# christoskokas/gtsam-vSLAM

Measured on AMD Instinct MI355X. Metric: frames/sec (extract+match+localBA), 1500 feat stereo 752x480, higher is better.
Workload: dtype u8/i32 (extract, match) + f64 (pose LM, local BA)

## Files before the change

gtsam-vslam_amd/csrc/ba.hip:

```cpp
#include "common.hpp"
#include "comm.hpp"
#include "dmath.hpp"
#include "ba_pool.hpp"
#include "ba_packed.hpp"
#include <algorithm>
#include <cmath>
#include <numeric>
#include <vector>
#include <atomic>
#include <condition_variable>
#include <functional>
#include <memory>
#include <mutex>
#include <thread>

namespace vslam {

struct BaEdge {
    int a, b, fa, fb;
    DPose measured;
    double r[6], Ja[36], Jb[36];
    double Haa[36], Hab[36], Hbb[36], ga[6], gb[6];
};

struct BaDev {
    int NF, Lp, F, K, NE, n;
    const int* facKf; const int* facFi; const int* facLp; const int* facLm;
    const double* facZ; const double* facIs; const uint8_t* facRight;
    double* facJ;
    const int* lpStart; const int* lpSlotStart; const int* slotStart; const int* slotFi; const int* lpOrig;
    DPose* poseCur; DPose* poseTrial; const int* fidx;
    double* lmCur; double* lmTrial;
    BaEdge* edges;
    double* S; double* rhs; double* Spart; double* Sedge; double* dP; double* dL;
    double* sums; double* partial;
    int* flags;
    double fx, fy, cx, cy, b;
    double* ctl;
    int NB, specLin, cand;
    int adaptive, nAct;
    double lambda;
    DPose* poseBase; double* lmBase; size_t lmStride;
    double* facJBase; size_t facJStride; double* SedgeBase; BaEdge* edgesBase;
    double* facJ2; double* Sedge2; BaEdge* edges2;
    size_t sysStride, spartStride, partialStride, dLStride;
    int solveKind;
    double* Lg;
    double* ctlHost;
};
enum { BA_SOLVE_MFMA64 = 0, BA_SOLVE_WAVE = 1, BA_SOLVE_MFMA = 2, BA_SOLVE_LARGE = 3 };

enum { CTL_LAMBDA = 0, CTL_ERROR = 1, CTL_CUR = 2, CTL_INIT_ERR = 3, CTL_INTS = 8, CTL_DOUBLES = 16 };
enum { CI_STATE = 0, CI_SEL = 1, CI_ITER = 2, CI_INNER = 3, CI_MAXIT = 4, CI_FIRST = 5, CI_NACT = 6, CI_ROUNDS = 7 };
enum { BA_LINEARIZE = 0, BA_TRY = 1, BA_DONE = 2 };
enum { BA_MAX_NB = 4, SUMS_CAND = 16, FLAG_COUNT = 1, FLAG_FAIL = 4 };
__device__ __forceinline__ int ba_slot(int sel, int c, int NB) {
    const int s = sel + 1 + c;
    return s > NB ? s - (NB + 1) : s;
}
__device__ __forceinline__ bool ba_enter(BaDev& D, int state, int c = 0) {
    const int* ci = (const int*)(D.ctl + CTL_INTS);
    if (ci[CI_STATE] != state) return false;
    D.nAct = ci[CI_NACT];
    if (c >= D.nAct) return false;
    const int sel = ci[CI_SEL], ts = ba_slot(sel, c, D.NB);
    D.cand = c;
    D.poseCur = D.poseBase + (size_t)sel * D.K; D.poseTrial = D.poseBase + (size_t)ts * D.K;
    D.lmCur = D.lmBase + (size_t)sel * D.lmStride; D.lmTrial = D.lmBase + (size_t)ts * D.lmStride;
    if (D.specLin) {
        const size_t se = (size_t)D.n * D.n + D.n;
        D.facJ = D.facJBase + (size_t)sel * D.facJStride; D.facJ2 = D.facJBase + (size_t)ts * D.facJStride;
        D.Sedge = D.SedgeBase + (size_t)sel * se; D.Sedge2 = D.SedgeBase + (size_t)ts * se;
        D.edges = D.edgesBase + (size_t)sel * D.NE; D.edges2 = D.edgesBase + (size_t)ts * D.NE;
    }
    D.S += (size_t)c * D.sysStride; D.rhs += (size_t)c * D.sysStride; D.Spart += (size_t)c * D.spartStride;
    D.dP += (size_t)c * D.n; D.dL += (size_t)c * D.dLStride; D.partial += (size_t)c * D.partialStride;
    double lam = D.ctl[CTL_LAMBDA];
    for (int i = 0; i < c; i++) lam *= 10.0;
    D.lambda = lam;
    return true;
}

constexpr int BA_SCHUR_WAVES = 16;
constexpr int BA_LDS_MAX_F = 20;
constexpr int BA_LDS_BYTES = 160 * 1024, BA_STATIC_LDS_RESERVE = 1024, BA_DYN_LDS_MAX = BA_LDS_BYTES - BA_STATIC_LDS_RESERVE;

__device__ __forceinline__ void ba_eval_fac(const BaDev& D, const DPose& T, const double* p, bool right,
                                            const double* z, double is, double* r, double* Jp, double* Jl) {
    const double d[3] = {p[0] - T.t[0], p[1] - T.t[1], p[2] - T.t[2]};
    double q[3];
    mat3T_vec(T.R, d, q);
    if (Jp) { for (int c = 0; c < 12; c++) Jp[c] = 0; for (int c = 0; c < 6; c++) Jl[c] = 0; }
    if (is == 0.0) { r[0] = r[1] = 0.0; return; }
    if (q[2] <= 0) { r[0] = r[1] = 2.0 * D.fx * is; return; }
    const double x = q[0], y = q[1], zz = q[2], iz = 1.0 / zz;
    const double xx = right ? x - D.b : x;
    r[0] = (D.fx * xx * iz + D.cx - z[0]) * is;
    r[1] = (D.fy * y * iz + D.cy - z[1]) * is;
    if (!Jp) return;
    const double al[2][3] = {{D.fx * iz, 0, -D.fx * xx * iz * iz}, {0, D.fy * iz, -D.fy * y * iz * iz}};
    const double Sk[3][3] = {{0, -zz, y}, {zz, 0, -x}, {-y, x, 0}};
    for (int a = 0; a < 2; a++)
        for (int c = 0; c < 3; c++) {
            Jp[a * 6 + c] = (al[a][0] * Sk[0][c] + al[a][1] * Sk[1][c] + al[a][2] * Sk[2][c]) * is;
            Jp[a * 6 + 3 + c] = -al[a][c] * is;
            Jl[a * 3 + c] = (al[a][0] * T.R[3 * c] + al[a][1] * T.R[3 * c + 1] + al[a][2] * T.R[3 * c + 2]) * is;
        }
}

__device__ __forceinline__ void ba_eval_edge(const BaEdge& e, const DPose& Ta, const DPose& Tb, double* r,
                                             double* Ja, double* Jb) {
    const double w = 1.0 / 0.01;
    DPose Tai, h, Mi, d;
    pose_inverse(Ta, Tai);
    pose_compose(Tai, Tb, h);
    pose_inverse(e.measured, Mi);
    pose_compose(Mi, h, d);
    pose3_logmap(d, r);
    for (int i = 0; i < 6; i++) r[i] *= w;
    if (!Ja) return;
    double Hl[36], Ad[36];
    DPose hi;
    pose3_logmap_derivative(d, Hl);
    pose_inverse(h, hi);
    pose3_adjoint(hi, Ad);
    for (int i = 0; i < 6; i++)
        for (int j = 0; j < 6; j++) {
            double s = 0;
            for (int k = 0; k < 6; k++) s += Hl[i * 6 + k] * Ad[k * 6 + j];
            Ja[i * 6 + j] = -s * w;
            Jb[i * 6 + j] = Hl[i * 6 + j] * w;
        }
}

__device__ __forceinline__ double ba_edge_linearize(BaEdge& out, const BaEdge& E, const DPose& Ta, const DPose& Tb,
                                                    double* sW, double* Sacc, int n, int tid) {
    double* Hl = sW; double* Ad = Hl + 36; double* Ja = Ad + 36; double* Jb = Ja + 36; double* rr = Jb + 36;
    const double w = 1.0 / 0.01;
    const int fa = E.fa, fb = E.fb;
    const int lane = tid & 63, wave = tid >> 6;
    double v = 0;
    if (lane == 0 && wave < 3) {
        DPose Tai, h;
        pose_inverse(Ta, Tai);
        pose_compose(Tai, Tb, h);
        if (wave == 2) {
            DPose hi;
            pose_inverse(h, hi);
            pose3_adjoint(hi, Ad);
        } else {
            DPose Mi, d;
            pose_inverse(E.measured, Mi);
            pose_compose(Mi, h, d);
            if (wave == 0) {
                double r[6];
                pose3_logmap(d, r);
                for (int i = 0; i < 6; i++) { r[i] *= w; rr[i] = r[i]; out.r[i] = r[i]; v += r[i] * r[i]; }
            } else pose3_logmap_derivative(d, Hl);
        }
    }
    __syncthreads();
    if (wave != 0) return 0.0;
    asm volatile("s_waitcnt lgkmcnt(0)" ::: "memory");
    const int i = lane / 6, j = lane % 6;
    if (lane < 36) {
// ... 45 lines not shown
    __syncthreads();
    if (tid < NV) {
        double s = 0;
        for (int w = 0; w < NW; w++) s += red[w * NV + tid];
        out[tid] = s;
    }
    __syncthreads();
}

__device__ __forceinline__ void ba_ctl(const BaDev& D, int mode, double relTol, double absTol) {
    double* c = D.ctl;
    int* ci = (int*)(D.ctl + CTL_INTS);
    if (mode == 0) {
        if (ci[CI_STATE] != BA_LINEARIZE) return;
        if (ci[CI_FIRST]) {
            ci[CI_FIRST] = 0;
            c[CTL_ERROR] = D.sums[0];
            c[CTL_INIT_ERR] = D.sums[0];
            ci[CI_STATE] = (!(c[CTL_ERROR] <= 0.0) && ci[CI_ITER] < ci[CI_MAXIT]) ? BA_TRY : BA_DONE;
        } else ci[CI_STATE] = BA_TRY;
        c[CTL_CUR] = c[CTL_ERROR];
        return;
    }
    if (ci[CI_STATE] != BA_TRY) return;
    ci[CI_ROUNDS]++;
    const int nAct = ci[CI_NACT];
    for (int cand = 0; cand < nAct; cand++) {
        const double error = c[CTL_ERROR];
        double lambda = c[CTL_LAMBDA];
        bool stepOk = false, stop = false;
        double newErr = INFINITY;
        const double linChange = error - D.sums[SUMS_CAND + 2 * cand];
        if (!D.flags[FLAG_FAIL + cand] && linChange >= 0) {
            newErr = D.sums[SUMS_CAND + 2 * cand + 1];
            const double costChange = error - newErr;
            if (linChange > DBL_EPSILON * error) stepOk = (costChange / linChange) > 1e-3;
            if (fabs(costChange) < relTol * error) stop = true;
        }
        bool endInner = false;
        if (stepOk) {
            ci[CI_SEL] = ba_slot(ci[CI_SEL], cand, D.NB);
            c[CTL_ERROR] = newErr;
            lambda = lambda / 10.0;
            c[CTL_LAMBDA] = lambda > 0.0 ? lambda : 0.0;
            ci[CI_ITER]++; ci[CI_INNER]++;
            endInner = true;
        } else if (!stop) {
            lambda *= 10.0;
            c[CTL_LAMBDA] = lambda;
            ci[CI_INNER]++;
            if (lambda >= 1e5) endInner = true;
        } else endInner = true;
        if (!endInner) continue;
        const double currentError = c[CTL_CUR], newError = c[CTL_ERROR];
        bool converged;
        if (newError <= 0.0) converged = true;
        else {
            const double absDec = currentError - newError, relDec = absDec / currentError;
            converged = (relDec <= relTol) || (absDec <= absTol);
        }
        ci[CI_STATE] = (ci[CI_ITER] < ci[CI_MAXIT] && !converged && isfinite(currentError)) ? BA_LINEARIZE : BA_DONE;
        if (D.specLin && ci[CI_STATE] == BA_LINEARIZE) {
            c[CTL_CUR] = c[CTL_ERROR];
            ci[CI_STATE] = BA_TRY;
        }
        ci[CI_NACT] = D.adaptive ? 1 : D.NB;
        return;
    }
    ci[CI_NACT] = D.NB;
}

__global__ __launch_bounds__(256) void k_ba_ctl(const BaDev* __restrict__ tab, int mode, double relTol, double absTol) {
    BaDev D = *lane_entry(tab, blockIdx.z);
    __shared__ int sZero;
    if (threadIdx.x == 0) {
        ba_ctl(D, mode, relTol, absTol);
        sZero = mode == 1 && ((const int*)(D.ctl + CTL_INTS))[CI_STATE] == BA_LINEARIZE;
    }
    __syncthreads();
    if (sZero) for (int i = threadIdx.x; i < D.n * D.n + D.n; i += 256) D.Sedge[i] = 0;
}

template <int MODE>
__global__ __launch_bounds__(256) void k_ba_factors(const BaDev* __restrict__ tab, int obsBlocks, int fuseCtl, double relTol, double absTol) {
    BaDev D = *lane_entry(tab, blockIdx.z);
    __shared__ double red[8], out[2];
    __shared__ double sW[160];
    __shared__ int sLast;
    double* const partialBase = D.partial;
    const int cand = MODE == 0 ? 0 : (int)blockIdx.y;
    const bool active = ba_enter(D, MODE == 0 ? BA_LINEARIZE : BA_TRY, cand);
    if (!active && ((const int*)(D.ctl + CTL_INTS))[CI_STATE] != (MODE == 0 ? BA_LINEARIZE : BA_TRY)) return;
    const int tid = threadIdx.x;
    if (!active) {
    } else if ((int)blockIdx.x < obsBlocks) {
        double v[2] = {0, 0};
        for (int f = blockIdx.x * 256 + tid; f < D.NF; f += obsBlocks * 256) {
            if (MODE == 0) {
                double r[2], Jp[12], Jl[6];
                ba_eval_fac(D, D.poseCur[D.facKf[f]], D.lmCur + 3 * (size_t)D.facLm[f], D.facRight[f], D.facZ + 2 * (size_t)f,
                            D.facIs[f], r, Jp, Jl);
                double* o = D.facJ + (size_t)f * 20;
                o[0] = r[0]; o[1] = r[1];
                for (int c = 0; c < 12; c++) o[2 + c] = Jp[c];
                for (int c = 0; c < 6; c++) o[14 + c] = Jl[c];
                v[0] += r[0] * r[0] + r[1] * r[1];
            } else {
                const double* o = D.facJ + (size_t)f * 20;
                const int fi = D.facFi[f], lp = D.facLp[f];
                double l0 = o[0], l1 = o[1];
                if (fi >= 0) {
                    const double* dp = D.dP + 6 * fi;
                    for (int i = 0; i < 6; i++) { l0 += o[2 + i] * dp[i]; l1 += o[8 + i] * dp[i]; }
                }
                const double* dl = D.dL + 3 * (size_t)lp;
                for (int i = 0; i < 3; i++) { l0 += o[14 + i] * dl[i]; l1 += o[17 + i] * dl[i]; }
                v[0] += l0 * l0 + l1 * l1;
                double r[2];
                if (D.specLin) {
                    double Jp[12], Jl[6];
                    ba_eval_fac(D, D.poseTrial[D.facKf[f]], D.lmTrial + 3 * (size_t)D.facLm[f], D.facRight[f], D.facZ + 2 * (size_t)f,
                                D.facIs[f], r, Jp, Jl);
                    double* o2 = D.facJ2 + (size_t)f * 20;
                    o2[0] = r[0]; o2[1] = r[1];
                    for (int c = 0; c < 12; c++) o2[2 + c] = Jp[c];
                    for (int c = 0; c < 6; c++) o2[14 + c] = Jl[c];
                } else
                    ba_eval_fac(D, D.poseTrial[D.facKf[f]], D.lmTrial + 3 * (size_t)D.facLm[f], D.facRight[f], D.facZ + 2 * (size_t)f,
                                D.facIs[f], r, nullptr, nullptr);
                v[1] += r[0] * r[0] + r[1] * r[1];
            }
        }
        ba_block_sum<2, 4>(v, red, out);
        if (tid == 0) { ba_publish(&D.partial[2 * blockIdx.x], out[0]); ba_publish(&D.partial[2 * blockIdx.x + 1], out[1]); }
    } else {
        const int e = blockIdx.x - obsBlocks;
        double v[2] = {0, 0};
        if (e < D.NE) {
            const BaEdge& E = D.edges[e];
            const int fa = E.fa, fb = E.fb;
            if (MODE == 0) {
                v[0] = ba_edge_linearize(D.edges[e], E, D.poseCur[E.a], D.poseCur[E.b], sW, D.Sedge, D.n, tid);
            } else {
                if (tid >= 8 && tid < 14) {
                    const int k = tid - 8;
                    double l = E.r[k];
                    for (int i = 0; i < 6; i++) {
                        if (fa >= 0) l += E.Ja[k * 6 + i] * D.dP[6 * fa + i];
                        if (fb >= 0) l += E.Jb[k * 6 + i] * D.dP[6 * fb + i];
                    }
                    v[0] += l * l;
                }
                if (D.specLin) v[1] = ba_edge_linearize(D.edges2[e], E, D.poseTrial[E.a], D.poseTrial[E.b], sW, D.Sedge2, D.n, tid);
                else if (tid == 0) {
                    DPose Tai, h, Mi, d;
                    pose_inverse(D.poseTrial[E.a], Tai);
                    pose_compose(Tai, D.poseTrial[E.b], h);
                    pose_inverse(E.measured, Mi);
                    pose_compose(Mi, h, d);
                    double r[6];
                    pose3_logmap(d, r);
                    for (int i = 0; i < 6; i++) { r[i] *= 1.0 / 0.01; v[1] += r[i] * r[i]; }
                }
            }
#pragma unroll
            for (int k = 0; k < 2; k++) {
#pragma unroll
                for (int d = 32; d >= 1; d >>= 1) v[k] += __shfl_xor(v[k], d);
// ... 4 lines not shown
    asm volatile("s_waitcnt vmcnt(0)" ::: "memory");
    __syncthreads();
    const int nCandRun = MODE == 0 ? 1 : D.nAct;
    if (tid == 0) sLast = (__hip_atomic_fetch_add(&D.flags[FLAG_COUNT], 1, __ATOMIC_RELAXED, __HIP_MEMORY_SCOPE_AGENT) == (int)(gridDim.x * gridDim.y) - 1);
    __syncthreads();
    if (!sLast) return;
    const int nPart = obsBlocks + D.NE;
    for (int c = 0; c < nCandRun; c++) {
        const double* part = partialBase + (size_t)c * D.partialStride;
        double t[2] = {0, 0};
        for (int i = tid; i < nPart; i += 256) { t[0] += ba_collect(&part[2 * i]); t[1] += ba_collect(&part[2 * i + 1]); }
        ba_block_sum<2, 4>(t, red, out);
        if (tid == 0) {
            if (MODE == 0) D.sums[0] = 0.5 * out[0];
            else { D.sums[SUMS_CAND + 2 * c] = 0.5 * out[0]; D.sums[SUMS_CAND + 2 * c + 1] = 0.5 * out[1]; }
        }
        __syncthreads();
    }
    if (tid == 0) {
        D.flags[FLAG_COUNT] = 0;
        sLast = 0;
        if (fuseCtl) {
            ba_ctl(D, MODE, relTol, absTol);
            sLast = MODE == 1 && !D.specLin && ((const int*)(D.ctl + CTL_INTS))[CI_STATE] == BA_LINEARIZE;
            if (D.ctlHost) {
                asm volatile("s_waitcnt vmcnt(0) lgkmcnt(0)" ::: "memory");
                const unsigned long long* src = (const unsigned long long*)D.ctl;
                unsigned long long* dst = (unsigned long long*)D.ctlHost;
                for (int i = 0; i < CTL_DOUBLES; i++) dst[i] = __hip_atomic_load(&src[i], __ATOMIC_RELAXED, __HIP_MEMORY_SCOPE_AGENT);
                __threadfence_system();
            }
        }
    }
    __syncthreads();
    if (sLast) for (int i = tid; i < D.n * D.n + D.n; i += 256) D.Sedge[i] = 0;
}

__device__ __forceinline__ void ba_wave_fence() { asm volatile("s_waitcnt lgkmcnt(0)" ::: "memory"); }

constexpr int BA_LPL_SCHUR = 64, BA_LPL_BACK = 32;
template <int BA_LPL>
__device__ __forceinline__ void ba_lm_blocks(const BaDev& D, int lp, bool act, double* W, int* sfi, double* h, int& ns) {
    const int lane = threadIdx.x & (BA_LPL - 1);
    const int f0 = act ? D.lpStart[lp] : 0, f1 = act ? D.lpStart[lp + 1] : 0;
#pragma unroll
    for (int k = 0; k < 9; k++) h[k] = 0;
    for (int f = f0 + lane; f < f1; f += BA_LPL) {
        const double* o = D.facJ + (size_t)f * 20;
        const double r0 = o[0], r1 = o[1];
        const double* Jl = o + 14;
        h[0] += Jl[0] * Jl[0] + Jl[3] * Jl[3];
        h[1] += Jl[0] * Jl[1] + Jl[3] * Jl[4];
        h[2] += Jl[0] * Jl[2] + Jl[3] * Jl[5];
        h[3] += Jl[1] * Jl[1] + Jl[4] * Jl[4];
        h[4] += Jl[1] * Jl[2] + Jl[4] * Jl[5];
        h[5] += Jl[2] * Jl[2] + Jl[5] * Jl[5];
        h[6] -= Jl[0] * r0 + Jl[3] * r1;
        h[7] -= Jl[1] * r0 + Jl[4] * r1;
        h[8] -= Jl[2] * r0 + Jl[5] * r1;
    }
#pragma unroll
    for (int k = 0; k < 9; k++) {
#pragma unroll
        for (int d = BA_LPL / 2; d >= 1; d >>= 1) h[k] += __shfl_xor(h[k], d);
    }
    const int s0 = act ? D.lpSlotStart[lp] : 0;
    ns = act ? D.lpSlotStart[lp + 1] - s0 - 1 : 0;
    for (int e = lane; e < ns * 18; e += BA_LPL) {
        const int s = e / 18, ij = e - s * 18, i = ij / 3, j = ij - i * 3;
        double acc = 0;
        for (int f = D.slotStart[s0 + s]; f < D.slotStart[s0 + s + 1]; f++) {
            const double* o = D.facJ + (size_t)f * 20;
            acc += o[2 + i] * o[14 + j] + o[2 + 6 + i] * o[14 + 3 + j];
        }
        W[e] = acc;
    }
    for (int s = lane; s < ns; s += BA_LPL) sfi[s] = D.slotFi[s0 + s];
}
__device__ __forceinline__ void ba_hll_inverse(const double* h, double lambda, double* Hi) {
    const double Hll[9] = {h[0] + lambda, h[1], h[2], h[1], h[3] + lambda, h[4], h[2], h[4], h[5] + lambda};
    inv3sym(Hll, Hi);
}

__global__ __launch_bounds__(64 * BA_SCHUR_WAVES) void k_ba_schur(const BaDev* __restrict__ tab, int maxSlots, int sharedW) {
    BaDev D = *lane_entry(tab, blockIdx.z);
    constexpr bool LDS_S = true;
    extern __shared__ double sm[];
    double* const SBase = D.S;
    double* const SpartBase = D.Spart;
    (void)SBase;
    const int c0 = sharedW ? 0 : (int)blockIdx.y;
    if (!ba_enter(D, BA_TRY, c0)) return;
    const int nc = sharedW ? D.nAct : 1;
    const int n = D.n;
    const size_t sys = (size_t)n * n + n;
    constexpr int BA_LPL = BA_LPL_SCHUR;
    double* Sloc = sm;
    double* wbase = sm + (LDS_S ? (size_t)nc * sys : 0);
    static_assert(BA_LPL == 64, "one wave per landmark: the landmark index is wave-uniform");
    const int lane = threadIdx.x & (BA_LPL - 1);
    const int unit = __builtin_amdgcn_readfirstlane(threadIdx.x / BA_LPL);
    double* W = wbase + (size_t)unit * (2 * maxSlots * 18);
    double* WH = W + maxSlots * 18;
    const int nu = blockDim.x / BA_LPL, nt = blockDim.x;
    int* sfi = (int*)(wbase + (size_t)nu * (2 * maxSlots * 18)) + unit * maxSlots;
    if (LDS_S) {
        for (int i = threadIdx.x; i < (int)(nc * sys); i += nt) Sloc[i] = 0;
    }
    __syncthreads();
    const int bi = lane / 6, bj = lane - bi * 6;
    const bool isBlk = lane < 36, isRhs = lane >= 36 && lane < 42;
    const int rr = isRhs ? lane - 36 : 0;
    const int hHalf = lane >= 27 ? 1 : 0, hq = lane - 27 * hHalf;
    const bool hRhs = hq >= 21;
    int hI = 0, hJ = 0;
    if (hRhs) hI = hq - 21;
    else { int rem = hq; while (rem >= 6 - hI) { rem -= 6 - hI; hI++; } hJ = hI + rem; }
    const int rounds = (D.Lp + gridDim.x * nu - 1) / (gridDim.x * nu);
    for (int rd = 0; rd < rounds; rd++) {
        const int lp = (rd * gridDim.x + blockIdx.x) * nu + unit;
        const bool act = lp < D.Lp;
        double h[9];
        int ns = 0;
        ba_lm_blocks<BA_LPL>(D, lp, act, W, sfi, h, ns);
        ba_wave_fence();
        double lamk = D.lambda;
        for (int k = 0; k < nc; k++, lamk *= 10.0) {
            double* Sacc = LDS_S ? Sloc + (size_t)k * sys : SBase + (size_t)(c0 + k) * D.sysStride;
            double* racc = Sacc + (size_t)n * n;
            double Hi[9];
            ba_hll_inverse(h, lamk, Hi);
            for (int e = lane; e < ns * 18; e += BA_LPL) {
                const int s = e / 18, ij = e - s * 18, i = ij / 3, j = ij - i * 3;
                const double* w = W + s * 18 + i * 3;
                WH[e] = w[0] * Hi[j] + w[1] * Hi[3 + j] + w[2] * Hi[6 + j];
            }
            ba_wave_fence();
            const int nsu = __builtin_amdgcn_readfirstlane(ns);
            for (int s1 = 0; s1 < nsu; s1++) {
                const int k1 = __builtin_amdgcn_readfirstlane(sfi[s1]);
                const double* a = WH + s1 * 18 + (isBlk ? bi : rr) * 3;
                const double a0 = a[0], a1 = a[1], a2 = a[2];
                if (isBlk) {
                    double* drow = Sacc + (size_t)(6 * k1 + bi) * n + bj;
                    for (int s2 = s1; s2 < nsu; s2++) {
                        const int k2 = __builtin_amdgcn_readfirstlane(sfi[s2]);
                        const double* bb = W + s2 * 18 + bj * 3;
                        atomicAdd(drow + 6 * k2, -(a0 * bb[0] + a1 * bb[1] + a2 * bb[2]));
                    }
                } else if (isRhs) atomicAdd(&racc[6 * k1 + rr], -(a0 * h[6] + a1 * h[7] + a2 * h[8]));
            }
            ba_wave_fence();
        }
        const int f0 = act ? D.lpStart[lp] : 0, f1 = act ? D.lpStart[lp + 1] : 0;
        if (lane < 54) {
            for (int f = f0 + hHalf; f < f1; f += 2) {
                const int fi = D.facFi[f];
                if (fi < 0) continue;
                const double* o = D.facJ + (size_t)f * 20;
                const double val = hRhs ? -(o[2 + hI] * o[0] + o[8 + hI] * o[1]) : o[2 + hI] * o[2 + hJ] + o[8 + hI] * o[8 + hJ];
                const size_t idx = hRhs ? (size_t)n * n + 6 * fi + hI : (size_t)(6 * fi + hI) * n + 6 * fi + hJ;
                for (int k = 0; k < nc; k++) atomicAdd((LDS_S ? Sloc + (size_t)k * sys : SBase + (size_t)(c0 + k) * D.sysStride) + idx, val);
            }
        }
    }
    if (LDS_S) {
        __syncthreads();
        for (int k = 0; k < nc; k++) {
// ... 31 lines not shown
};
struct Ba2Region { double* F; double* W; double* WH; double* hb; int* ffi; int* sst; int* sfi; };
__device__ __forceinline__ Ba2Region ba2_region(double* base, int maxFac, int maxSlots) {
    Ba2Region g;
    g.F = base; g.W = g.F + maxFac * 20; g.WH = g.W + maxSlots * 18; g.hb = g.WH + maxSlots * 18;
    g.ffi = (int*)(g.hb + 10); g.sst = g.ffi + maxFac; g.sfi = g.sst + maxSlots + 1;
    return g;
}
__device__ __forceinline__ void ba2_stage_h(const BaDev& D, int lp, const Ba2Region& g, const Ba2Roles& R, int lane, double* h, int& nf, int& ns) {
    const int f0 = D.lpStart[lp], s0 = D.lpSlotStart[lp];
    nf = D.lpStart[lp + 1] - f0;
    ns = D.lpSlotStart[lp + 1] - s0 - 1;
    {
        const double2* src = (const double2*)(D.facJ + (size_t)f0 * 20);
        double2* dst = (double2*)g.F;
        for (int i = lane; i < nf * 10; i += 64) dst[i] = src[i];
        for (int i = lane; i < nf; i += 64) g.ffi[i] = D.facFi[f0 + i];
        for (int i = lane; i <= ns; i += 64) { g.sst[i] = D.slotStart[s0 + i] - f0; g.sfi[i] = D.slotFi[s0 + i]; }
    }
    ba_wave_fence();
    {
        double acc = 0;
        if (R.hOn)
            for (int f = R.hq; f < nf; f += 4) {
                const double* o = g.F + f * 20;
                acc += o[R.hx] * o[R.hy] + o[R.hx + 3] * o[R.hy + R.hyStep];
            }
        acc += ba2_dpp_xor(acc, 0);
        acc += ba2_dpp_xor(acc, 1);
        if (R.hOn && R.hq == 0) g.hb[R.hk] = R.hSign * acc;
    }
    ba_wave_fence();
#pragma unroll
    for (int k = 0; k < 9; k++) h[k] = g.hb[k];
}
__device__ __forceinline__ void ba2_w_row(const Ba2Region& g, const Ba2Roles& R, double& w0, double& w1, double& w2) {
    w0 = w1 = w2 = 0;
    for (int f = g.sst[R.ws]; f < g.sst[R.ws + 1]; f++) {
        const double* o = g.F + f * 20;
        const double a0 = o[2 + R.wi], a1 = o[8 + R.wi];
        w0 += a0 * o[14] + a1 * o[17];
        w1 += a0 * o[15] + a1 * o[18];
        w2 += a0 * o[16] + a1 * o[19];
    }
}

enum { BA2_ROWMAJOR = 0, BA2_ROWMAJOR1 = 1, BA2_PACKED = 2 };
__host__ __device__ inline int ba2_sys_doubles(int n, int layout) {
    return layout == BA2_PACKED ? (ba_packed_doubles(n / 6) + 1) & ~1 : layout == BA2_ROWMAJOR1 ? n * (n + 1) + n : n * n + n;
}
__host__ __device__ inline int ba2_part_doubles(int n, int layout) {
    return layout == BA2_PACKED ? ba_packed_doubles(n / 6) : n * n + n;
}
template <bool PACKED>
__device__ __forceinline__ void ba2_blocks(double* Sloc, const double* W, const double* WH, const int* sfi, int ns, int lane, int F, int ld) {
    const int nb = ns * (ns + 1) / 2, half = lane & 1;
    for (int b0 = 0; b0 < nb; b0 += 32) {
        int b = b0 + (lane >> 1), s1 = 0;
        if (b >= nb) continue;
        while (b >= ns - s1) { b -= ns - s1; s1++; }
        const int s2 = s1 + b;
        const double* A = WH + s1 * 18 + half * 9;
        const double* B = W + s2 * 18;
        double aa[9];
#pragma unroll
        for (int q = 0; q < 9; q++) aa[q] = A[q];
        double* d0 = Sloc + (PACKED ? ba_packed_block(F, sfi[s1], sfi[s2]) * BA_PACKED_PITCH + 18 * half : (6 * sfi[s1] + 3 * half) * ld + 6 * sfi[s2]);
#pragma unroll
        for (int jh = 0; jh < 2; jh++) {
            double bb[9];
#pragma unroll
            for (int q = 0; q < 9; q++) bb[q] = B[9 * jh + q];
#pragma unroll
            for (int i = 0; i < 3; i++) {
                double* dr = d0 + i * (PACKED ? 6 : ld) + 3 * jh;
#pragma unroll
                for (int j = 0; j < 3; j++) atomicAdd(dr + j, -(aa[3 * i] * bb[3 * j] + aa[3 * i + 1] * bb[3 * j + 1] + aa[3 * i + 2] * bb[3 * j + 2]));
            }
        }
    }
}

template <bool PACKED>
__device__ __forceinline__ void ba2_schur(const BaDev* __restrict__ tab, int maxSlots, int maxFac, int layout) {
    BaDev D = *lane_entry(tab, blockIdx.z);
    extern __shared__ double sm[];
    if (!ba_enter(D, BA_TRY, blockIdx.y)) return;
    const int n = D.n, F = n / 6;
    constexpr bool packed = PACKED;
    const int ld = layout == BA2_ROWMAJOR1 ? n + 1 : n;
    const int sys = ba2_sys_doubles(n, layout);
    double* const Sloc = sm;
    double* const racc = Sloc + (packed ? ba_packed_rhs(F) : ld * n);
    const int lane = threadIdx.x & 63;
    const int unit = __builtin_amdgcn_readfirstlane(threadIdx.x >> 6), nu = blockDim.x >> 6, nt = blockDim.x;
    const Ba2Region g = ba2_region(sm + sys + (size_t)unit * ba2_stage_doubles(maxFac, maxSlots), maxFac, maxSlots);
    double* const F_ = g.F; double* const W = g.W; double* const WH = g.WH;
    int* const ffi = g.ffi; int* const sfi = g.sfi;
    const double lam = D.lambda;
    Ba2Roles R;
    R.init(lane);
    const int pf = lane / 6, pi = lane - pf * 6;
    for (int i = threadIdx.x; i < sys; i += nt) Sloc[i] = 0;
    __syncthreads();
    for (int lp = blockIdx.x * nu + unit; lp < D.Lp; lp += gridDim.x * nu) {
        double h[9];
        int nf, ns;
        ba2_stage_h(D, lp, g, R, lane, h, nf, ns);
        double Hi[9];
        ba_hll_inverse(h, lam, Hi);
        if (R.ws < ns) {
            double w0, w1, w2;
            ba2_w_row(g, R, w0, w1, w2);
            const double g0 = w0 * Hi[0] + w1 * Hi[3] + w2 * Hi[6], g1 = w0 * Hi[1] + w1 * Hi[4] + w2 * Hi[7], g2 = w0 * Hi[2] + w1 * Hi[5] + w2 * Hi[8];
            double* wr = W + R.ws * 18 + R.wi * 3;
            wr[0] = w0; wr[1] = w1; wr[2] = w2;
            double* gr = WH + R.ws * 18 + R.wi * 3;
            gr[0] = g0; gr[1] = g1; gr[2] = g2;
            atomicAdd(&racc[6 * sfi[R.ws] + R.wi], -(g0 * h[6] + g1 * h[7] + g2 * h[8]));
        }
        ba_wave_fence();
        ba2_blocks<PACKED>(Sloc, W, WH, sfi, ns, lane, F, ld);
        if (pf < 10)
            for (int fb = 0; fb < nf; fb += 10) {
                const int f = fb + pf;
                if (f >= nf) break;
                const int fi = ffi[f];
                if (fi < 0) continue;
                const double* o = F_ + f * 20;
                const double a0 = o[2 + pi], a1 = o[8 + pi];
                double* dr = Sloc + (packed ? ba_packed_block(F, fi, fi) * BA_PACKED_PITCH + 6 * pi : (6 * fi + pi) * ld + 6 * fi);
                for (int j = pi; j < 6; j++) atomicAdd(dr + j, a0 * o[2 + j] + a1 * o[8 + j]);
                atomicAdd(&racc[6 * fi + pi], -(a0 * o[0] + a1 * o[1]));
            }
        ba_wave_fence();
    }
    __syncthreads();
    const int part = ba2_part_doubles(n, layout);
    double* dst = D.Spart + (size_t)blockIdx.x * part;
    if (layout == BA2_ROWMAJOR1) {
        for (int i = threadIdx.x; i < part; i += nt) dst[i] = Sloc[i + i / n];
    } else {
        for (int i = threadIdx.x; i < part; i += nt) dst[i] = Sloc[i];
    }
}
__global__ __launch_bounds__(1024) void k_ba_schur2(const BaDev* __restrict__ tab, int maxSlots, int maxFac) { ba2_schur<true>(tab, maxSlots, maxFac, BA2_PACKED); }
__global__ __launch_bounds__(1024) void k_ba_schur2_rm(const BaDev* __restrict__ tab, int maxSlots, int maxFac, int layout) { ba2_schur<false>(tab, maxSlots, maxFac, layout); }

__global__ __launch_bounds__(512) void k_ba_back2(const BaDev* __restrict__ tab, int maxSlots, int maxFac) {
    BaDev D = *lane_entry(tab, blockIdx.z);
    extern __shared__ double sm[];
    if (!ba_enter(D, BA_TRY, 0)) return;
    const int nc = D.nAct;
    const int sel = ((const int*)(D.ctl + CTL_INTS))[CI_SEL];
    const int lane = threadIdx.x & 63;
    const int unit = __builtin_amdgcn_readfirstlane(threadIdx.x >> 6), nu = blockDim.x >> 6;
    const Ba2Region g = ba2_region(sm + (size_t)unit * ba2_stage_doubles(maxFac, maxSlots), maxFac, maxSlots);
    Ba2Roles R;
    R.init(lane);
    for (int lp = blockIdx.x * nu + unit; lp < D.Lp; lp += gridDim.x * nu) {
        double h[9];
        int nf, ns;
        ba2_stage_h(D, lp, g, R, lane, h, nf, ns);
        double w0 = 0, w1 = 0, w2 = 0;
        int kcol = 0;
        if (R.ws < ns) { ba2_w_row(g, R, w0, w1, w2); kcol = 6 * g.sfi[R.ws] + R.wi; }
        const int l = D.lpOrig[lp];
        double lamk = D.lambda;
        for (int k = 0; k < nc; k++, lamk *= 10.0) {
            const double* dPk = D.dP + (size_t)k * D.n;
            const double dp = R.ws < ns ? dPk[kcol] : 0.0;
            double t0 = w0 * dp, t1 = w1 * dp, t2 = w2 * dp;
            t0 += ba2_dpp_xor(t0, 0); t1 += ba2_dpp_xor(t1, 0); t2 += ba2_dpp_xor(t2, 0);
            t0 += ba2_dpp_xor(t0, 1); t1 += ba2_dpp_xor(t1, 1); t2 += ba2_dpp_xor(t2, 1);
#pragma unroll
            for (int d = 4; d <= 32; d <<= 1) { t0 += __shfl_xor(t0, d); t1 += __shfl_xor(t1, d); t2 += __shfl_xor(t2, d); }
            double Hi[9];
            ba_hll_inverse(h, lamk, Hi);
            if (lane < 3) {
                const double u0 = h[6] - t0, u1 = h[7] - t1, u2 = h[8] - t2;
                const double h0 = lane == 0 ? Hi[0] : (lane == 1 ? Hi[3] : Hi[6]);
                const double h1 = lane == 0 ? Hi[1] : (lane == 1 ? Hi[4] : Hi[7]);
                const double h2 = lane == 0 ? Hi[2] : (lane == 1 ? Hi[5] : Hi[8]);
                const double dl = h0 * u0 + h1 * u1 + h2 * u2;
                D.dL[(size_t)k * D.dLStride + 3 * (size_t)lp + lane] = dl;
                double* lmT = D.lmBase + (size_t)ba_slot(sel, k, D.NB) * D.lmStride;
                lmT[3 * (size_t)l + lane] = D.lmCur[3 * (size_t)l + lane] + dl;
            }
        }
        ba_wave_fence();
    }
}

__global__ __launch_bounds__(256) void k_ba_reduce(const BaDev* __restrict__ tab, int nPart, int packed) {
    BaDev D = *lane_entry(tab, blockIdx.z);
    __shared__ double sSl[8][33];
    if (!ba_enter(D, BA_TRY, blockIdx.y)) return;
    const int total = D.n * D.n + D.n, F = D.n / 6;
    const int nSum = packed ? ba_packed_doubles(F) : total;
    const int nSlots = packed ? ba_packed_reduce_slots(F) : total;
    const int e = threadIdx.x & 31, y = threadIdx.x >> 5;
    const int i = blockIdx.x * 32 + e;
    double s = 0;
    if (i < nSum) {
        const int per = (nPart + 7) / 8;
        const int p0 = y * per, p1 = min(nPart, p0 + per);
        double s0 = 0, s1 = 0, s2 = 0, s3 = 0;
        int p = p0;
        for (; p + 3 < p1; p += 4) {
            s0 += D.Spart[p * nSum + i];
            s1 += D.Spart[(p + 1) * nSum + i];
            s2 += D.Spart[(p + 2) * nSum + i];
            s3 += D.Spart[(p + 3) * nSum + i];
        }
        for (; p < p1; p++) s0 += D.Spart[p * nSum + i];
        s = (s0 + s1) + (s2 + s3);
    }
    sSl[y][e] = s;
    __syncthreads();
    const int slot = blockIdx.x * 32 + threadIdx.x;
    if (y == 0 && slot < nSlots) {
        const int io = packed ? ba_packed_reduce_entry(F, slot) : slot;
        if (io >= 0) {
            double t = D.Sedge[io];
            for (int q = 0; q < 8; q++) t += sSl[q][threadIdx.x];
            if (D.specLin) D.Sedge2[io] = 0;
            if (io < D.n * D.n) D.S[io] = t; else D.rhs[io - D.n * D.n] = t;
        }
    }
}

struct BaWin {
    int TB, T, TP, tileDoubles, nWin;
    const int* winA; const int* winB;
    const int* winFirstWg;
    const int* wgWin; const int* wgBegin; const int* wgEnd;
    const int* winLm;
    double* part;
    double* Wg; double* Hg;
};

constexpr int BA_WIN_HG = 9 + 6 * BA_MAX_NB;
__global__ __launch_bounds__(64 * BA_SCHUR_WAVES) void k_ba_lm_prep(const BaDev* __restrict__ tab, BaWin Wn, int maxSlots) {
    BaDev D = *lane_entry(tab, blockIdx.z);
    extern __shared__ int smi[];
    if (!ba_enter(D, BA_TRY, 0)) return;
    constexpr int BA_LPL = 64;
    const int lane = threadIdx.x & 63, unit = threadIdx.x >> 6, nu = blockDim.x >> 6;
    int* sfi = smi + unit * maxSlots;
    for (int lp = blockIdx.x * nu + unit; lp < D.Lp; lp += gridDim.x * nu) {
        double h[9];
        int ns = 0;
        ba_lm_blocks<BA_LPL>(D, lp, true, Wn.Wg + (size_t)D.lpSlotStart[lp] * 18, sfi, h, ns);
        double* Hl = Wn.Hg + (size_t)lp * BA_WIN_HG;
        if (lane < 9) {
            double v = h[0];
#pragma unroll
            for (int k = 1; k < 9; k++) if (lane == k) v = h[k];
            Hl[lane] = v;
        } else if (lane >= 16 && lane < 16 + D.nAct) {
            double lamk = D.lambda;
            for (int k = 16; k < lane; k++) lamk *= 10.0;
            double Hi[9];
            ba_hll_inverse(h, lamk, Hi);
            double* o = Hl + 9 + 6 * (lane - 16);
            o[0] = Hi[0]; o[1] = Hi[1]; o[2] = Hi[2]; o[3] = Hi[4]; o[4] = Hi[5]; o[5] = Hi[8];
        }
    }
}

constexpr int BA_WIN_META = 5 * 64 + 65;
__global__ __launch_bounds__(64 * BA_SCHUR_WAVES) void k_ba_schur_win(const BaDev* __restrict__ tab, BaWin Wn) {
    BaDev D = *lane_entry(tab, blockIdx.z);
    extern __shared__ double sm[];
    if (!ba_enter(D, BA_TRY, 0)) return;
    const int nc = D.nAct, T = Wn.T, TP = Wn.TP, tile = Wn.tileDoubles;
    const int win = Wn.wgWin[blockIdx.x], wa = Wn.winA[win], wb = Wn.winB[win];
    const int r0 = wa * Wn.TB, r1 = min(D.F, r0 + Wn.TB), c0 = wb * Wn.TB, c1 = min(D.F, c0 + Wn.TB);
    const bool diag = wa == wb;
    double* Sloc = sm;
    const int lane = threadIdx.x & 63, wave = threadIdx.x >> 6, nw = blockDim.x >> 6, nt = blockDim.x;
    int* meta = (int*)(sm + (size_t)nc * tile) + wave * BA_WIN_META;
    int* mLp = meta; int* mSeR = meta + 64; int* mNR = meta + 128; int* mSeC = meta + 192; int* mNC = meta + 256; int* pref = meta + 320;
    for (int i = threadIdx.x; i < nc * tile; i += nt) Sloc[i] = 0;
    __syncthreads();
    const int i0 = Wn.wgBegin[blockIdx.x], i1 = Wn.wgEnd[blockIdx.x];
    const int g = lane / 6, ri = lane - 6 * g;
    for (int base = i0 + wave * 64; base < i1; base += nw * 64) {
        {
            const int idx = base + lane;
            const bool valid = idx < i1;
            const int lp = valid ? Wn.winLm[idx] : 0;
            const int se0 = valid ? D.lpSlotStart[lp] : 0;
            const int ns = valid ? D.lpSlotStart[lp + 1] - se0 - 1 : 0;
            int sr0 = ns, sr1 = 0, sc0 = ns, sc1 = 0;
            for (int q = 0; q < ns; q++) {
                const int fi = D.slotFi[se0 + q];
                if (fi >= r0 && fi < r1) { sr0 = min(sr0, q); sr1 = q + 1; }
                if (fi >= c0 && fi < c1) { sc0 = min(sc0, q); sc1 = q + 1; }
            }
            const int nr = max(sr1 - sr0, 0), ncs = max(sc1 - sc0, 0);
            const int np = (nr > 0 && ncs > 0) ? (diag ? nr * (nr + 1) / 2 : nr * ncs) : 0;
            int incl = np;
#pragma unroll
            for (int d = 1; d < 64; d <<= 1) { const int t = __shfl_up(incl, d); if (lane >= d) incl += t; }
            mLp[lane] = lp; mSeR[lane] = se0 + sr0; mNR[lane] = nr; mSeC[lane] = se0 + sc0; mNC[lane] = ncs;
            pref[lane] = incl - np;
            if (lane == 63) pref[64] = incl;
        }
        ba_wave_fence();
        const int P = pref[64];
// ... 170 lines not shown
#pragma unroll
            for (int c = 0; c < 6; c++) {
                double v = ri[J + c];
#pragma unroll
                for (int m = 0; m < c; m++) v -= x[m] * Ld[c][m];
                x[c] = v * inv[c];
            }
        }
        __syncthreads();
        if (bad) { if (tid == 0) sFail = 1; break; }
        if (tid > J + 5 && tid < n) {
#pragma unroll
            for (int c = 0; c < 6; c++) A[(size_t)tid * ld + J + c] = x[c];
        } else if (tid >= J && tid < J + 6) {
            const int r = tid - J;
#pragma unroll
            for (int c = 0; c < 6; c++) if (c <= r) A[(size_t)tid * ld + J + c] = Ld[r][c];
            idiag[tid] = inv[r];
        }
        __syncthreads();
    }
    __syncthreads();
    BA_STAMP(3)
    if (!sFail) {
        double* bv = rhsl;
        for (int J = 0; J < n; J += 6) {
            double y[6];
#pragma unroll
            for (int c = 0; c < 6; c++) {
                double v = bv[J + c];
#pragma unroll
                for (int m = 0; m < c; m++) v -= A[(size_t)(J + c) * ld + J + m] * y[m];
                y[c] = v * idiag[J + c];
            }
            if (tid > J + 5 && tid < n) {
                const double* ri = A + (size_t)tid * ld + J;
                double v = bv[tid];
#pragma unroll
                for (int c = 0; c < 6; c++) v -= ri[c] * y[c];
                bv[tid] = v;
            }
            if (tid == J) {
#pragma unroll
                for (int c = 0; c < 6; c++) col[J + c] = y[c];
            }
            __syncthreads();
        }
        BA_STAMP(4)
        for (int J = n - 6; J >= 0; J -= 6) {
            double x[6];
#pragma unroll
            for (int c = 5; c >= 0; c--) {
                double v = col[J + c];
#pragma unroll
                for (int m = 5; m > c; m--) v -= A[(size_t)(J + m) * ld + J + c] * x[m];
                x[c] = v * idiag[J + c];
            }
            __syncthreads();
            if (tid < J) {
                double v = col[tid];
#pragma unroll
                for (int c = 0; c < 6; c++) v -= A[(size_t)(J + c) * ld + tid] * x[c];
                col[tid] = v;
            }
            if (tid == J) {
#pragma unroll
                for (int c = 0; c < 6; c++) D.dP[J + c] = x[c];
            }
            __syncthreads();
        }
        BA_STAMP(5)
        for (int k = tid; k < D.K; k += nt) {
            const int fi = D.fidx[k];
            if (fi >= 0) { DPose T; pose_retract(D.poseCur[k], D.dP + 6 * fi, T); D.poseTrial[k] = T; }
            else D.poseTrial[k] = D.poseCur[k];
        }
    }
    __syncthreads();
    BA_STAMP(6)
    if (tid == 0) D.flags[FLAG_FAIL + D.cand] = sFail;
}

constexpr int BA_WAVE_N = 60;
__global__ __launch_bounds__(64) void k_ba_solve_wave(const BaDev* __restrict__ tab) {
    BaDev D = *lane_entry(tab, blockIdx.z);
    constexpr int N = BA_WAVE_N;
    __shared__ double Lt[N * (N + 1)];
    if (D.solveKind != BA_SOLVE_WAVE) return;
    if (!ba_enter(D, BA_TRY, blockIdx.x)) return;
    const double lambda = D.lambda;
    const int n = D.n, lane = threadIdx.x;
    const int r = lane < N ? lane : N - 1;
    double a[N];
#ifdef VSLAM_BA_STAMPS
#define BAW_STAMP(i) if (lane == 0) D.sums[8 + (i)] = (double)__builtin_readcyclecounter();
#else
#define BAW_STAMP(i)
#endif
    BAW_STAMP(0)
    for (int row = 0; row < n; row++)
        if (lane < n) Lt[row * (N + 1) + lane] = D.S[(size_t)row * n + lane];
    asm volatile("s_waitcnt vmcnt(0) lgkmcnt(0)" ::: "memory");
#pragma unroll
    for (int c = 0; c < N; c++) {
        double v = (c == r) ? 1.0 : 0.0;
        if (r < n && c < n) v = Lt[r <= c ? r * (N + 1) + c : c * (N + 1) + r] + ((c == r) ? lambda : 0.0);
        a[c] = v;
    }
    asm volatile("s_waitcnt lgkmcnt(0)" ::: "memory");
    double b = r < n ? D.rhs[r] : 0.0;
    bool bad = false;
    BAW_STAMP(1)
    BAW_STAMP(2)
    double idg = 1.0;
#pragma unroll
    for (int k = 0; k < N; k++) {
        double d = readlane_d(a[k], k);
        if (!(d > 0)) { bad = true; d = 1.0; }
        const double id = rsqrt(d);
        const double lk = (r == k) ? d * id : a[k] * id;
        if (r == k) idg = id;
        a[k] = lk;
#pragma unroll
        for (int j = k + 1; j < N; j++) a[j] = __builtin_fma(-lk, readlane_d(lk, j), a[j]);
    }
    BAW_STAMP(3)
    if (!bad) {
#pragma unroll
        for (int k = 0; k < N; k++) {
            const double yk = readlane_d(b, k) * readlane_d(idg, k);
            if (r == k) b = yk; else if (r > k) b -= a[k] * yk;
        }
        BAW_STAMP(4)
        if (lane < N) {
#pragma unroll
            for (int j = 0; j < N; j++) Lt[lane * (N + 1) + j] = a[j];
        }
        asm volatile("s_waitcnt lgkmcnt(0)" ::: "memory");
#pragma unroll
        for (int k = 0; k < N; k++) a[k] = Lt[k * (N + 1) + r];
#pragma unroll
        for (int k = N - 1; k >= 0; k--) {
            const double xk = readlane_d(b, k) * readlane_d(idg, k);
            if (r == k) b = xk; else if (r < k) b -= a[k] * xk;
        }
        BAW_STAMP(5)
        if (lane < n) D.dP[lane] = b;
        Lt[lane] = b;
        asm volatile("s_waitcnt lgkmcnt(0)" ::: "memory");
        for (int k = lane; k < D.K; k += 64) {
            const int fi = D.fidx[k];
            if (fi >= 0) { DPose T; pose_retract(D.poseCur[k], Lt + 6 * fi, T); D.poseTrial[k] = T; }
            else D.poseTrial[k] = D.poseCur[k];
        }
    }
    BAW_STAMP(6)
    if (lane == 0) D.flags[FLAG_FAIL + D.cand] = bad ? 1 : 0;
}

constexpr int BA_MFMA_N = 256, BA_MFMA_NB = BA_MFMA_N / 16, BA_MFMA_NW = 8, BA_MFMA_SLOTS = 17, BA_MFMA_LD = 17;
typedef double ba_d4 __attribute__((ext_vector_type(4)));

__global__ __launch_bounds__(64 * BA_MFMA_NW) void k_ba_solve_mfma(const BaDev* __restrict__ tab, double* __restrict__ Lg) {
    BaDev D = *lane_entry(tab, blockIdx.z);
    extern __shared__ double sm[];
    double* P = sm;
    double* sInv = P + BA_MFMA_N * BA_MFMA_LD;
    double* sB = sInv + 16;
    __shared__ int sBad;
    if (D.solveKind != BA_SOLVE_MFMA) return;
    if (!ba_enter(D, BA_TRY, blockIdx.x)) return;
    const double lambda = D.lambda;
    constexpr int N = BA_MFMA_N, NB = BA_MFMA_NB, LD = BA_MFMA_LD;
    if (D.Lg) Lg = D.Lg;
    Lg += (size_t)D.cand * N * N;
    const int n = D.n, tid = threadIdx.x, lane = tid & 63;
    const int wave = __builtin_amdgcn_readfirstlane(tid >> 6);
    if (tid == 0) sBad = 0;
    ba_d4 acc[BA_MFMA_SLOTS];
    int tpk[BA_MFMA_SLOTS];
#pragma unroll
    for (int s = 0; s < BA_MFMA_SLOTS; s++) {
        const int t = s * BA_MFMA_NW + wave;
        int ib = 0;
        while ((ib + 1) * (ib + 2) / 2 <= t) ib++;
        const int jb = t - ib * (ib + 1) / 2;
        const bool valid = ib < NB;
        tpk[s] = (valid ? ib : 255) | (jb << 8);
#pragma unroll
        for (int r = 0; r < 4; r++) {
            const int row = ib * 16 + (lane >> 4) + 4 * r, col = jb * 16 + (lane & 15);
            double v = (row == col) ? 1.0 : 0.0;
            if (valid && row < n && col < n) v = D.S[(size_t)col * n + row] + ((row == col) ? lambda : 0.0);
            acc[s][r] = v;
        }
    }
    for (int i = tid; i < N; i += 64 * BA_MFMA_NW) sB[i] = i < n ? D.rhs[i] : 0.0;
    __syncthreads();
    for (int kb = 0; kb < NB; kb++) {
#pragma unroll
        for (int s = 0; s < BA_MFMA_SLOTS; s++) {
            const int tib = tpk[s] & 255, tjb = tpk[s] >> 8;
            if (tib != 255 && tib >= kb && tjb == kb) {
#pragma unroll
                for (int r = 0; r < 4; r++) P[(tib * 16 + (lane >> 4) + 4 * r) * LD + (lane & 15)] = acc[s][r];
            }
        }
        __syncthreads();
        if (wave == 0) {
            const int r = lane & 15;
            double a[16];
#pragma unroll
            for (int c = 0; c < 16; c++) a[c] = P[(kb * 16 + r) * LD + c];
            bool bad = false;
            double idg = 1.0;
#pragma unroll
            for (int k = 0; k < 16; k++) {
                double d = readlane_d(a[k], k);
                if (!(d > 0)) { bad = true; d = 1.0; }
                const double id = rsqrt(d);
                const double lk = (r == k) ? d * id : a[k] * id;
                if (r == k) idg = id;
                a[k] = lk;
#pragma unroll
                for (int j = k + 1; j < 16; j++) a[j] = __builtin_fma(-lk, readlane_d(lk, j), a[j]);
            }
            if (lane < 16) {
#pragma unroll
                for (int c = 0; c < 16; c++) P[(kb * 16 + r) * LD + c] = a[c];
                sInv[r] = idg;
            }
            if (bad && lane == 0) sBad = 1;
        }
        __syncthreads();
        for (int row = (kb + 1) * 16 + tid; row < N; row += 64 * BA_MFMA_NW) {
            double x[16];
#pragma unroll
            for (int c = 0; c < 16; c++) {
                double v = P[row * LD + c];
#pragma unroll
                for (int m = 0; m < c; m++) v = __builtin_fma(-x[m], P[(kb * 16 + c) * LD + m], v);
                x[c] = v * sInv[c];
            }
#pragma unroll
            for (int c = 0; c < 16; c++) { P[row * LD + c] = x[c]; Lg[(size_t)row * N + kb * 16 + c] = x[c]; }
        }
        if (tid < 16) {
#pragma unroll
            for (int c = 0; c < 16; c++) Lg[(size_t)(kb * 16 + tid) * N + kb * 16 + c] = c <= tid ? P[(kb * 16 + tid) * LD + c] : 0.0;
        }
        __syncthreads();
#pragma unroll
        for (int s = 0; s < BA_MFMA_SLOTS; s++) {
            const int tib = tpk[s] & 255, tjb = tpk[s] >> 8;
            if (tib != 255 && tib > kb && tjb > kb) {
                const double* pa = P + (tib * 16 + (lane & 15)) * LD + (lane >> 4);
                const double* pb = P + (tjb * 16 + (lane & 15)) * LD + (lane >> 4);
#pragma unroll
                for (int ks = 0; ks < 4; ks++) acc[s] = __builtin_amdgcn_mfma_f64_16x16x4f64(-pa[4 * ks], pb[4 * ks], acc[s], 0, 0, 0);
            }
        }
        __syncthreads();
    }
    const bool fail = sBad != 0;
    if (!fail) {
        __threadfence_block();
        for (int kb = 0; kb < NB; kb++) {
            if (wave == 0) {
                const int r = lane & 15;
                double b = sB[kb * 16 + r];
                double lrow[16];
#pragma unroll
                for (int c = 0; c < 16; c++) lrow[c] = Lg[(size_t)(kb * 16 + r) * N + kb * 16 + c];
#pragma unroll
                for (int k = 0; k < 16; k++) {
                    const double yk = readlane_d(b, k) / readlane_d(lrow[k], k);
                    if (r == k) b = yk; else if (r > k) b = __builtin_fma(-lrow[k], yk, b);
                }
                if (lane < 16) sB[kb * 16 + r] = b;
            }
            __syncthreads();
            for (int row = (kb + 1) * 16 + tid; row < N; row += 64 * BA_MFMA_NW) {
                double v = sB[row];
                const double* lr = Lg + (size_t)row * N + kb * 16;
#pragma unroll
                for (int c = 0; c < 16; c++) v = __builtin_fma(-lr[c], sB[kb * 16 + c], v);
                sB[row] = v;
            }
            __syncthreads();
        }
        for (int kb = NB - 1; kb >= 0; kb--) {
            if (wave == 0) {
                const int r = lane & 15;
                double b = sB[kb * 16 + r];
                double lcol[16];
#pragma unroll
                for (int c = 0; c < 16; c++) lcol[c] = Lg[(size_t)(kb * 16 + c) * N + kb * 16 + r];
#pragma unroll
                for (int k = 15; k >= 0; k--) {
                    const double xk = readlane_d(b, k) / readlane_d(lcol[k], k);
                    if (r == k) b = xk; else if (r < k) b = __builtin_fma(-lcol[k], xk, b);
                }
                if (lane < 16) sB[kb * 16 + r] = b;
            }
            __syncthreads();
            for (int row = tid; row < kb * 16; row += 64 * BA_MFMA_NW) {
                double v = sB[row];
#pragma unroll
                for (int c = 0; c < 16; c++) v = __builtin_fma(-Lg[(size_t)(kb * 16 + c) * N + row], sB[kb * 16 + c], v);
                sB[row] = v;
            }
            __syncthreads();
        }
        for (int i = tid; i < n; i += 64 * BA_MFMA_NW) D.dP[i] = sB[i];
        for (int k = tid; k < D.K; k += 64 * BA_MFMA_NW) {
            const int fi = D.fidx[k];
            if (fi >= 0) { DPose T; pose_retract(D.poseCur[k], sB + 6 * fi, T); D.poseTrial[k] = T; }
            else D.poseTrial[k] = D.poseCur[k];
        }
    }
    if (tid == 0) D.flags[FLAG_FAIL + D.cand] = fail ? 1 : 0;
}

__global__ __launch_bounds__(64) void k_ba_solve_mfma64(const BaDev* __restrict__ tab) {
    BaDev D = *lane_entry(tab, blockIdx.z);
    constexpr int N = 64, LDF = 65, LD = 17;
    __shared__ double Lf[N * LDF];
    __shared__ double P[N * LD];
    __shared__ double sInv[16], sB[N];
    if (D.solveKind != BA_SOLVE_MFMA64) return;
    if (!ba_enter(D, BA_TRY, blockIdx.x)) return;
    const double lambda = D.lambda;
    const int n = D.n, lane = threadIdx.x;
    auto fence = []() { asm volatile("s_waitcnt lgkmcnt(0)" ::: "memory"); };
    for (int row = 0; row < n; row++)
        if (lane < n) Lf[row * LDF + lane] = D.S[(size_t)row * n + lane];
    sB[lane] = lane < n ? D.rhs[lane] : 0.0;
    asm volatile("s_waitcnt vmcnt(0) lgkmcnt(0)" ::: "memory");
    ba_d4 acc[10];
#pragma unroll
    for (int ib = 0; ib < 4; ib++)
#pragma unroll
        for (int jb = 0; jb <= ib; jb++) {
            const int s = ib * (ib + 1) / 2 + jb;
#pragma unroll
            for (int r = 0; r < 4; r++) {
                const int row = ib * 16 + (lane >> 4) + 4 * r, col = jb * 16 + (lane & 15);
                double v = (row == col) ? 1.0 : 0.0;
                if (row < n && col < n) v = (row >= col ? Lf[col * LDF + row] : Lf[row * LDF + col]) + ((row == col) ? lambda : 0.0);
                acc[s][r] = v;
            }
        }
    fence();
    bool bad = false;
#pragma unroll
    for (int kb = 0; kb < 4; kb++) {
#pragma unroll
        for (int ib = kb; ib < 4; ib++) {
            const int s = ib * (ib + 1) / 2 + kb;
#pragma unroll
            for (int r = 0; r < 4; r++) P[(ib * 16 + (lane >> 4) + 4 * r) * LD + (lane & 15)] = acc[s][r];
        }
        fence();
        {
            const int r = lane & 15;
            double a[16];
#pragma unroll
            for (int c = 0; c < 16; c++) a[c] = P[(kb * 16 + r) * LD + c];
            double idg = 1.0;
#pragma unroll
            for (int k = 0; k < 16; k++) {
                double d = readlane_d(a[k], k);
                if (!(d > 0)) { bad = true; d = 1.0; }
                const double id = rsqrt(d);
                const double lk = (r == k) ? d * id : a[k] * id;
                if (r == k) idg = id;
                a[k] = lk;
#pragma unroll
                for (int j = k + 1; j < 16; j++) a[j] = __builtin_fma(-lk, readlane_d(lk, j), a[j]);
            }
            if (lane < 16) {
#pragma unroll
                for (int c = 0; c < 16; c++) { P[(kb * 16 + r) * LD + c] = a[c]; Lf[(kb * 16 + r) * LDF + kb * 16 + c] = c <= r ? a[c] : 0.0; }
                sInv[r] = idg;
            }
        }
        fence();
        {
            const int row = (kb + 1) * 16 + lane;
            if (row < N) {
                double x[16];
#pragma unroll
                for (int c = 0; c < 16; c++) {
                    double v = P[row * LD + c];
#pragma unroll
                    for (int m = 0; m < c; m++) v = __builtin_fma(-x[m], P[(kb * 16 + c) * LD + m], v);
                    x[c] = v * sInv[c];
                }
#pragma unroll
                for (int c = 0; c < 16; c++) { P[row * LD + c] = x[c]; Lf[row * LDF + kb * 16 + c] = x[c]; }
            }
        }
        fence();
#pragma unroll
        for (int ib = kb + 1; ib < 4; ib++)
#pragma unroll
            for (int jb = kb + 1; jb <= ib; jb++) {
                const int s = ib * (ib + 1) / 2 + jb;
                const double* pa = P + (ib * 16 + (lane & 15)) * LD + (lane >> 4);
                const double* pb = P + (jb * 16 + (lane & 15)) * LD + (lane >> 4);
#pragma unroll
                for (int ks = 0; ks < 4; ks++) acc[s] = __builtin_amdgcn_mfma_f64_16x16x4f64(-pa[4 * ks], pb[4 * ks], acc[s], 0, 0, 0);
            }
        fence();
    }
    if (!bad) {
        const double inv = 1.0 / Lf[lane * LDF + lane];
        double b = sB[lane];
#pragma unroll 8
        for (int k = 0; k < N; k++) {
            const double lik = Lf[lane * LDF + k];
            const double yk = readlane_d(b, k) * readlane_d(inv, k);
            if (lane == k) b = yk; else if (lane > k) b = __builtin_fma(-lik, yk, b);
        }
#pragma unroll 8
        for (int k = N - 1; k >= 0; k--) {
            const double lki = Lf[k * LDF + lane];
            const double xk = readlane_d(b, k) * readlane_d(inv, k);
            if (lane == k) b = xk; else if (lane < k) b = __builtin_fma(-lki, xk, b);
        }
        if (lane < n) D.dP[lane] = b;
        sB[lane] = b;
        fence();
        for (int k = lane; k < D.K; k += 64) {
            const int fi = D.fidx[k];
            if (fi >= 0) { DPose T; pose_retract(D.poseCur[k], sB + 6 * fi, T); D.poseTrial[k] = T; }
            else D.poseTrial[k] = D.poseCur[k];
        }
    }
    if (lane == 0) D.flags[FLAG_FAIL + D.cand] = bad ? 1 : 0;
}

constexpr int CH_B = 64, CH_LD = 65, CH_PLD = 17;

__global__ __launch_bounds__(256) void k_ba_chol_col(const BaDev* __restrict__ tab, double* __restrict__ Lg, double* __restrict__ yG, int N, int J, int* __restrict__ failFlag) {
    BaDev D = *lane_entry(tab, blockIdx.z);
    extern __shared__ double sm[];
    double* sA = sm;
    double* sB = sA + CH_B * CH_LD;
    double* sP = sB + CH_B * CH_LD;
    double* sInv = sP + CH_B * CH_PLD;
    double* sT = sInv + CH_B;
    double* sY = sT + CH_B;
    __shared__ int sBad;
    if (!ba_enter(D, BA_TRY, blockIdx.y)) return;
    const double lambda = D.lambda;
    const int n = D.n, tid = threadIdx.x, lane = tid & 63, wave = tid >> 6;
    const int I = J + (int)blockIdx.x;
    const bool isDiag = blockIdx.x == 0;
    Lg += (size_t)D.cand * N * N; yG += (size_t)D.cand * N;
    if (tid == 0) sBad = 0;
    auto Aij = [&](int i, int j) -> double {
        if (i >= n || j >= n) return i == j ? 1.0 : 0.0;
        return D.S[i <= j ? (size_t)i * n + j : (size_t)j * n + i] + (i == j ? lambda : 0.0);
    };
    ba_d4 accC[4], accD[4];
#pragma unroll
    for (int cb = 0; cb < 4; cb++)
#pragma unroll
        for (int r = 0; r < 4; r++) {
            const int lr = 16 * wave + (lane >> 4) + 4 * r, lc = cb * 16 + (lane & 15);
            accD[cb][r] = Aij(J * CH_B + lr, J * CH_B + lc);
            accC[cb][r] = isDiag ? 0.0 : Aij(I * CH_B + lr, J * CH_B + lc);
        }
    double t = 0;
    if (isDiag && tid < CH_B) t = (J * CH_B + tid) < n ? D.rhs[J * CH_B + tid] : 0.0;
    for (int K = 0; K < J; K++) {
        __syncthreads();
        for (int e = tid; e < CH_B * CH_B; e += 256) {
            const int r = e >> 6, c = e & 63;
            sB[r * CH_LD + c] = Lg[(size_t)(J * CH_B + r) * N + K * CH_B + c];
            if (!isDiag) sA[r * CH_LD + c] = Lg[(size_t)(I * CH_B + r) * N + K * CH_B + c];
        }
        if (isDiag && tid < CH_B) sY[tid] = yG[K * CH_B + tid];
        __syncthreads();
        const double* pd = sB + (16 * wave + (lane & 15)) * CH_LD + (lane >> 4);
        const double* pa = sA + (16 * wave + (lane & 15)) * CH_LD + (lane >> 4);
#pragma unroll
        for (int cb = 0; cb < 4; cb++) {
            const double* pb = sB + (cb * 16 + (lane & 15)) * CH_LD + (lane >> 4);
#pragma unroll
            for (int ks = 0; ks < 16; ks++) {
                const double b = pb[4 * ks];
                if (cb <= wave) accD[cb] = __builtin_amdgcn_mfma_f64_16x16x4f64(-pd[4 * ks], b, accD[cb], 0, 0, 0);
                if (!isDiag) accC[cb] = __builtin_amdgcn_mfma_f64_16x16x4f64(-pa[4 * ks], b, accC[cb], 0, 0, 0);
            }
        }
        if (isDiag && tid < CH_B) {
            const double* lr = sB + tid * CH_LD;
            double a0 = 0, a1 = 0;
#pragma unroll 8
            for (int c = 0; c < CH_B; c += 2) { a0 += lr[c] * sY[c]; a1 += lr[c + 1] * sY[c + 1]; }
            t -= a0 + a1;
        }
    }
    __syncthreads();
    for (int e = tid; e < CH_B * CH_LD; e += 256) sB[e] = 0.0;
    __syncthreads();
#pragma unroll
    for (int kb = 0; kb < 4; kb++) {
        if (wave >= kb) {
#pragma unroll
            for (int r = 0; r < 4; r++) sP[(wave * 16 + (lane >> 4) + 4 * r) * CH_PLD + (lane & 15)] = accD[kb][r];
        }
        __syncthreads();
        if (wave == 0) {
            const int r = lane & 15;
            double a[16];
#pragma unroll
            for (int c = 0; c < 16; c++) a[c] = sP[(kb * 16 + r) * CH_PLD + c];
            bool bad = false;
            double idg = 1.0;
#pragma unroll
// ... 65 lines not shown
        }
        return;
    }
    double* X = sA + (size_t)(16 * wave) * CH_LD;
#pragma unroll
    for (int cb = 0; cb < 4; cb++) {
#pragma unroll
        for (int r = 0; r < 4; r++) X[((lane >> 4) + 4 * r) * CH_LD + cb * 16 + (lane & 15)] = accC[cb][r];
        ba_wave_fence();
        if (lane < 16) {
            double x[16];
#pragma unroll
            for (int c = 0; c < 16; c++) {
                double v = X[lane * CH_LD + cb * 16 + c];
#pragma unroll
                for (int m = 0; m < c; m++) v = __builtin_fma(-x[m], sB[(cb * 16 + c) * CH_LD + cb * 16 + m], v);
                x[c] = v * sInv[cb * 16 + c];
            }
#pragma unroll
            for (int c = 0; c < 16; c++) X[lane * CH_LD + cb * 16 + c] = x[c];
        }
        ba_wave_fence();
        const double* pa = X + (lane & 15) * CH_LD + cb * 16 + (lane >> 4);
#pragma unroll
        for (int c2 = 1; c2 < 4; c2++) {
            if (c2 > cb) {
                const double* pb = sB + (c2 * 16 + (lane & 15)) * CH_LD + cb * 16 + (lane >> 4);
#pragma unroll
                for (int ks = 0; ks < 4; ks++) accC[c2] = __builtin_amdgcn_mfma_f64_16x16x4f64(-pa[4 * ks], pb[4 * ks], accC[c2], 0, 0, 0);
            }
        }
    }
    ba_wave_fence();
    for (int e = lane; e < 16 * CH_B; e += 64) {
        const int r = e >> 6, c = e & 63;
        Lg[(size_t)(I * CH_B + 16 * wave + r) * N + J * CH_B + c] = X[r * CH_LD + c];
    }
}

__global__ __launch_bounds__(256) void k_ba_chol_back(const BaDev* __restrict__ tab, const double* __restrict__ Lg, const double* __restrict__ yG, int N, int* __restrict__ failFlag) {
    BaDev D = *lane_entry(tab, blockIdx.z);
    extern __shared__ double sm[];
    double* sL = sm;
    double* sX = sL + CH_B * CH_LD;
    double* sR = sX + N;
    if (!ba_enter(D, BA_TRY, blockIdx.x)) return;
    const int n = D.n, tid = threadIdx.x, lane = tid & 63, wave = tid >> 6;
    Lg += (size_t)D.cand * N * N; yG += (size_t)D.cand * N;
    const bool fail = failFlag[D.cand] != 0;
    __syncthreads();
    if (tid == 0) { D.flags[FLAG_FAIL + D.cand] = fail ? 1 : 0; failFlag[D.cand] = 0; }
    if (fail) return;
    const int NBk = N / CH_B;
    for (int J = NBk - 1; J >= 0; J--) {
        double acc = 0;
        for (int i = (J + 1) * CH_B + wave; i < N; i += 4) acc += Lg[(size_t)i * N + J * CH_B + lane] * sX[i];
        sR[wave * CH_B + lane] = acc;
        for (int e = tid; e < CH_B * CH_B; e += 256) {
            const int r = e >> 6, c = e & 63;
            sL[r * CH_LD + c] = Lg[(size_t)(J * CH_B + r) * N + J * CH_B + c];
        }
        __syncthreads();
        if (wave == 0) {
            double b = yG[J * CH_B + lane] - ((sR[lane] + sR[CH_B + lane]) + (sR[2 * CH_B + lane] + sR[3 * CH_B + lane]));
            const double inv = 1.0 / sL[lane * CH_LD + lane];
#pragma unroll 8
            for (int k = CH_B - 1; k >= 0; k--) {
                const double lki = sL[k * CH_LD + lane];
                const double xk = readlane_d(b, k) * readlane_d(inv, k);
                if (lane == k) b = xk; else if (lane < k) b = __builtin_fma(-lki, xk, b);
            }
            sX[J * CH_B + lane] = b;
        }
        __syncthreads();
    }
    for (int i = tid; i < n; i += 256) D.dP[i] = sX[i];
    for (int k = tid; k < D.K; k += 256) {
        const int fi = D.fidx[k];
        if (fi >= 0) { DPose T; pose_retract(D.poseCur[k], sX + 6 * fi, T); D.poseTrial[k] = T; }
        else D.poseTrial[k] = D.poseCur[k];
    }
}

__global__ __launch_bounds__(64 * BA_SCHUR_WAVES) void k_ba_back(const BaDev* __restrict__ tab, int maxSlots, int allCand) {
    BaDev D = *lane_entry(tab, blockIdx.z);
    extern __shared__ double sm[];
    const int c0 = allCand ? 0 : (int)blockIdx.y;
    if (!ba_enter(D, BA_TRY, c0)) return;
    const int nc = allCand ? D.nAct : 1;
    const int sel = ((const int*)(D.ctl + CTL_INTS))[CI_SEL];
    constexpr int BA_LPL = BA_LPL_BACK;
    const int lane = threadIdx.x & (BA_LPL - 1), unit = threadIdx.x / BA_LPL;
    double* W = sm + (size_t)unit * (maxSlots * 18);
    const int nu = blockDim.x / BA_LPL;
    int* sfi = (int*)(sm + (size_t)nu * (maxSlots * 18)) + unit * maxSlots;
    const int rounds = (D.Lp + gridDim.x * nu - 1) / (gridDim.x * nu);
    for (int rd = 0; rd < rounds; rd++) {
        const int lp = (rd * gridDim.x + blockIdx.x) * nu + unit;
        const bool act = lp < D.Lp;
        double h[9];
        int ns = 0;
        ba_lm_blocks<BA_LPL>(D, lp, act, W, sfi, h, ns);
        ba_wave_fence();
        const int l = act ? D.lpOrig[lp] : 0;
        double lamk = D.lambda;
        for (int k = 0; k < nc; k++, lamk *= 10.0) {
            const double* dPk = D.dP + (size_t)k * D.n;
            double Hi[9];
            ba_hll_inverse(h, lamk, Hi);
            double t[3] = {0, 0, 0};
            for (int e = lane; e < ns * 6; e += BA_LPL) {
                const int s = e / 6, i = e - s * 6;
                const double dp = dPk[6 * sfi[s] + i];
                const double* w = W + s * 18 + i * 3;
                t[0] += w[0] * dp; t[1] += w[1] * dp; t[2] += w[2] * dp;
            }
#pragma unroll
            for (int q = 0; q < 3; q++) {
#pragma unroll
                for (int d = BA_LPL / 2; d >= 1; d >>= 1) t[q] += __shfl_xor(t[q], d);
            }
            if (act && lane < 3) {
                const double u[3] = {h[6] - t[0], h[7] - t[1], h[8] - t[2]};
                const double h0 = lane == 0 ? Hi[0] : (lane == 1 ? Hi[3] : Hi[6]);
                const double h1 = lane == 0 ? Hi[1] : (lane == 1 ? Hi[4] : Hi[7]);
                const double h2 = lane == 0 ? Hi[2] : (lane == 1 ? Hi[5] : Hi[8]);
                const double dl = h0 * u[0] + h1 * u[1] + h2 * u[2];
                D.dL[(size_t)k * D.dLStride + 3 * (size_t)lp + lane] = dl;
                double* lmT = D.lmBase + (size_t)ba_slot(sel, c0 + k, D.NB) * D.lmStride;
                lmT[3 * (size_t)l + lane] = D.lmCur[3 * (size_t)l + lane] + dl;
            }
        }
        ba_wave_fence();
    }
}

struct BaChi {
    int NP; const int* pairKf; const int* pairLm; const uint8_t* pairFlags; const float* pairUv; const int* pairOct;
    const uint8_t* kfLocal; const uint8_t* kfPresent; const uint8_t* lmPresent; const DPose* pose; const double* lm;
    float thr[MAX_LEVELS]; double fx, fy, cx, cy, b; uint8_t* wrong;
};
__device__ __forceinline__ bool ba_outlier(const BaChi& C, const double* pc, float ou, float ov, int oct, bool right) {
    const double x = right ? pc[0] - C.b : pc[0], y = pc[1], z = pc[2];
    if (z <= 0) return true;
    const double px = C.fx * x + C.cx * z, py = C.fy * y + C.cy * z;
    const double eu = (double)ou - px / z, ev = (double)ov - py / z;
    return (eu * eu + ev * ev) > (double)C.thr[oct];
}
__global__ __launch_bounds__(256) void k_ba_chi2(BaChi C) {
    const int p = blockIdx.x * 256 + threadIdx.x;
    if (p >= C.NP) return;
    uint8_t w = 0;
    const int kf = C.pairKf[p], lm = C.pairLm[p], fl = C.pairFlags[p];
    if (C.kfLocal[kf] && C.kfPresent[kf] && C.lmPresent[lm] && (fl & 3)) {
        DPose Tcw;
        pose_inverse(C.pose[kf], Tcw);
        double pc[3];
        mat3_vec(Tcw.R, C.lm + 3 * (size_t)lm, pc);
        for (int i = 0; i < 3; i++) pc[i] += Tcw.t[i];
        const float* uv = C.pairUv + 4 * (size_t)p;
        if (fl & 1) {
            if (ba_outlier(C, pc, uv[0], uv[1], C.pairOct[2 * p], false)) w = 1;
            else if ((fl & 2) && ba_outlier(C, pc, uv[2], uv[3], C.pairOct[2 * p + 1], true)) w = 1;
        } else if (ba_outlier(C, pc, uv[2], uv[3], C.pairOct[2 * p + 1], true)) w = 1;
    }
    C.wrong[p] = w;
}

// ... 1037 lines not shown
                for (int i0 = winCnt[w]; i0 < winCnt[w + 1]; i0 += chunk) { wgWin.push_back(w); wgBegin.push_back(i0); wgEnd.push_back(std::min(i0 + chunk, winCnt[w + 1])); }
            }
            winFirst[nWin] = (int)wgWin.size();
            nWinWg = (int)wgWin.size();
            const size_t nInts = (size_t)2 * nWin + (nWin + 1) + (size_t)3 * std::max(nWinWg, 1) + std::max(total, 1);
            std::vector<int> pack;
            pack.reserve(nInts);
            pack.insert(pack.end(), winA.begin(), winA.end()); pack.insert(pack.end(), winB.begin(), winB.end());
            pack.insert(pack.end(), winFirst.begin(), winFirst.end());
            const size_t oWg = pack.size();
            pack.insert(pack.end(), wgWin.begin(), wgWin.end()); pack.resize(oWg + std::max(nWinWg, 1));
            pack.insert(pack.end(), wgBegin.begin(), wgBegin.end()); pack.resize(oWg + 2 * (size_t)std::max(nWinWg, 1));
            pack.insert(pack.end(), wgEnd.begin(), wgEnd.end()); pack.resize(oWg + 3 * (size_t)std::max(nWinWg, 1));
            pack.insert(pack.end(), winLm.begin(), winLm.end());
            VS_HIP(d_win.alloc(nInts));
            VS_HIP(hipMemcpyAsync(d_win.p, pack.data(), pack.size() * sizeof(int), hipMemcpyHostToDevice, stream));
            if (devOrder && Q.nBlk > 0 && total > 0) {
                Q.winLm = d_win.p + oWg + 3 * (size_t)std::max(nWinWg, 1);
                hipLaunchKernelGGL(k_win_lists<1>, dim3(Q.nBlk), dim3(256), 0, stream, Q);
                VS_HIP(hipGetLastError());
            }
            VS_HIP(hipStreamSynchronize(stream));
            Wn.winA = d_win.p; Wn.winB = d_win.p + nWin; Wn.winFirstWg = d_win.p + 2 * nWin;
            Wn.wgWin = d_win.p + oWg; Wn.wgBegin = Wn.wgWin + std::max(nWinWg, 1); Wn.wgEnd = Wn.wgBegin + std::max(nWinWg, 1);
            Wn.winLm = Wn.wgEnd + std::max(nWinWg, 1);
            VS_HIP(d_Spart.alloc((size_t)std::max(nWinWg, 1) * NB * Wn.tileDoubles));
            Wn.part = d_Spart.p;
            VS_HIP(ws->d_winW.alloc((size_t)std::max(nSlotEntries, 1) * 18)); VS_HIP(ws->d_winH.alloc((size_t)std::max(Lp, 1) * BA_WIN_HG));
            Wn.Wg = ws->d_winW.p; Wn.Hg = ws->d_winH.p;
            VS_HIP(hipMemsetAsync(d_S.p, 0, sysStride * NB * sizeof(double), stream));
        }
        const int schurUnits = schurWaves * SCHUR_LPW;
        const int lmBlocks = std::max(1, std::min((Lp + schurUnits - 1) / schurUnits, nCU));
        int backWaves = BA_SCHUR_WAVES / BACK_LPW;
        { static const int cap = getenv("VSLAM_BA_BACK_WAVES") ? std::max(1, atoi(getenv("VSLAM_BA_BACK_WAVES"))) : 64; backWaves = std::min(backWaves, cap); }
        auto back_lds = [&](int nw) { return (size_t)nw * BACK_LPW * maxSlots * 18 * sizeof(double) + (size_t)nw * BACK_LPW * maxSlots * sizeof(int) + 16; };
        while (backWaves > 1 && back_lds(backWaves) > 150 * 1024) backWaves /= 2;
        const int backBlocks = std::max(1, std::min((Lp + backWaves * BACK_LPW - 1) / (backWaves * BACK_LPW), nCU));
        D.partialStride = (size_t)2 * obsBlocks + 2 * (size_t)std::max(NE, 1);
        VS_HIP(d_partial.alloc(D.partialStride * NB));
        D.partial = d_partial.p;
        D.spartStride = sysDoubles * lmBlocks;
        if (ldsS) { VS_HIP(d_Spart.alloc(D.spartStride * NB)); D.Spart = d_Spart.p; }
        const size_t backLds = back_lds(backWaves);
        const int sharedBack = (NB > 1 && sharedEnv) ? 1 : 0;
        const int ldA = ((n + 31) / 32) * 32 + 1;
        const size_t solveLdsBytes = ((size_t)n * ldA + n + 8) * sizeof(double);
        const bool solveLds = solveLdsBytes <= 150 * 1024;
#ifndef VSLAM_HOST_STAMPS
        BHS("u_alloc");
#endif
        if (n > 1024) { set_error("local BA: more than 170 free keyframes is not supported"); return VSLAM_ERR_CAPACITY; }
        if (schurLds > 160 * 1024) { set_error("local BA: landmark with too many views for the LDS staging"); return VSLAM_ERR_CAPACITY; }
        VS_CHECK(ba_kernel_attributes());
        const size_t mfmaLds = ((size_t)BA_MFMA_N * BA_MFMA_LD + 16 + BA_MFMA_N) * sizeof(double);
        const bool useMfma = ba_use_mfma();
        if (n > BA_WAVE_N && n <= BA_MFMA_N && useMfma) {
            VS_HIP(d_Lg.alloc((size_t)BA_MFMA_N * BA_MFMA_N * NB));
        }
        const bool useChol = n > BA_MFMA_N && useMfma;
        const int cholN = vslam::align_up(std::max(n, 1), CH_B);
        const size_t cholColLds = ((size_t)2 * CH_B * CH_LD + (size_t)CH_B * CH_PLD + 3 * CH_B) * sizeof(double);
        const size_t cholBackLds = ((size_t)CH_B * CH_LD + cholN + 4 * CH_B) * sizeof(double);
        if (useChol) {
            VS_HIP(d_Lg.alloc((size_t)cholN * cholN * NB));
            VS_HIP(d_cholY.alloc((size_t)cholN * NB));
            if (!d_cholFail.p) { VS_HIP(d_cholFail.alloc(BA_MAX_NB)); VS_HIP(hipMemsetAsync(d_cholFail.p, 0, BA_MAX_NB * sizeof(int), stream)); }
        }
#ifndef VSLAM_HOST_STAMPS
        BHS("u_attr");
#endif
        D.solveKind = (n <= 64 && useMfma) ? BA_SOLVE_MFMA64 : n <= BA_WAVE_N ? BA_SOLVE_WAVE : (n <= BA_MFMA_N && useMfma) ? BA_SOLVE_MFMA : BA_SOLVE_LARGE;
        *h_D = D;
        const BaDev* const dD = A.dev(h_D);
        VS_HIP(hipMemcpyAsync((void*)dD, h_D, sizeof(BaDev), hipMemcpyHostToDevice, stream));
        BHS("upload");

        auto run_lm = [&](int ps, long long nfStat, long long lpStat, long long k2Stat) -> vslam_status {
        (void)poseOut; (void)lmOut;
        const int fuseCtl = comm ? 0 : 1;
        const int facBlocks = (NF ? obsBlocks : 0) + std::max(NE, 1);
        const int nObs = NF ? obsBlocks : 0;
        VS_HIP(hipMemsetAsync(d_Sedge.p, 0, ((size_t)n * n + n) * sizeof(double), stream));
        auto step = [&](bool first) -> vslam_status {
            int t = -1;
            if (first || !specLin) {
                t = g_baTimer.begin("ba_linearize");
                hipLaunchKernelGGL(k_ba_factors<0>, dim3(facBlocks), dim3(256), 0, stream, dD, nObs, fuseCtl, relTol, absTol);
                g_baTimer.end(t);
            }
            if (comm) {
                const int tc = g_baTimer.begin("ba_allreduce"); VS_CHECK(comm_allreduce(comm, d_sums.p, 1, stream)); g_baTimer.end(tc);
                hipLaunchKernelGGL(k_ba_ctl, dim3(1), dim3(256), 0, stream, dD, 0, relTol, absTol);
            }
            t = g_baTimer.begin("ba_schur");
            if (n > 0) {
                if (ldsS) hipLaunchKernelGGL(k_ba_schur, dim3(lmBlocks, sharedW ? 1 : NB), dim3(64 * schurWaves), schurLds, stream, dD, maxSlots, sharedW);
                else if (nWinWg) {
                    hipLaunchKernelGGL(k_ba_lm_prep, dim3(std::max(1, std::min((Lp + BA_SCHUR_WAVES - 1) / BA_SCHUR_WAVES, 4 * nCU))), dim3(64 * BA_SCHUR_WAVES),
                                       (size_t)BA_SCHUR_WAVES * maxSlots * sizeof(int), stream, dD, Wn, maxSlots);
                    hipLaunchKernelGGL(k_ba_schur_win, dim3(nWinWg), dim3(64 * schurWaves), schurLds, stream, dD, Wn);
                }
            }
            g_baTimer.end(t);
            t = g_baTimer.begin("ba_solve");
            if (n > 0) {
                if (ldsS) hipLaunchKernelGGL(k_ba_reduce, dim3(((int)sysDoubles + 31) / 32, NB), dim3(256), 0, stream, dD, lmBlocks, 0);
                else hipLaunchKernelGGL(k_ba_reduce_win, dim3(Wn.nWin, NB), dim3(256), 0, stream, dD, Wn);
            }
            if (comm && n > 0) { const int tc = g_baTimer.begin("ba_allreduce"); VS_CHECK(comm_allreduce(comm, d_S.p, sysStride * (NB - 1) + (size_t)n * n + n, stream)); g_baTimer.end(tc); }
            if (n <= 64 && useMfma) hipLaunchKernelGGL(k_ba_solve_mfma64, dim3(NB), dim3(64), 0, stream, dD);
            else if (n <= BA_WAVE_N) hipLaunchKernelGGL(k_ba_solve_wave, dim3(NB), dim3(64), 0, stream, dD);
            else if (n <= BA_MFMA_N && useMfma) hipLaunchKernelGGL(k_ba_solve_mfma, dim3(NB), dim3(64 * BA_MFMA_NW), mfmaLds, stream, dD, d_Lg.p);
            else if (useChol) {
                for (int J = 0; J < cholN / CH_B; J++)
                    hipLaunchKernelGGL(k_ba_chol_col, dim3(cholN / CH_B - J, NB), dim3(256), cholColLds, stream, dD, d_Lg.p, d_cholY.p, cholN, J, d_cholFail.p);
                hipLaunchKernelGGL(k_ba_chol_back, dim3(NB), dim3(256), cholBackLds, stream, dD, (const double*)d_Lg.p, (const double*)d_cholY.p, cholN, d_cholFail.p);
            } else hipLaunchKernelGGL(k_ba_solve, dim3(NB), dim3(std::max(64, vslam::align_up(n, 64))),
                                    solveLds ? solveLdsBytes : 64, stream, dD, solveLds ? 1 : 0, solveLds ? ldA : n);
            g_baTimer.end(t);
            t = g_baTimer.begin("ba_back");
            if (Lp) hipLaunchKernelGGL(k_ba_back, dim3(backBlocks, sharedBack ? 1 : NB), dim3(64 * backWaves), backLds, stream, dD, maxSlots, sharedBack);
            g_baTimer.end(t);
            t = g_baTimer.begin("ba_eval");
            hipLaunchKernelGGL(k_ba_factors<1>, dim3(facBlocks, NB), dim3(256), 0, stream, dD, nObs, fuseCtl, relTol, absTol);
            g_baTimer.end(t);
            if (comm) {
                const int tc = g_baTimer.begin("ba_allreduce"); VS_CHECK(comm_allreduce(comm, d_sums.p + SUMS_CAND, (size_t)2 * NB, stream)); g_baTimer.end(tc);
                hipLaunchKernelGGL(k_ba_ctl, dim3(1), dim3(256), 0, stream, dD, 1, relTol, absTol);
            }
            VS_HIP(hipGetLastError());
            return VSLAM_OK;
        };
        double* h_ctlOut = ws->h_ctlOut;
        const int* co = (const int*)(h_ctlOut + CTL_INTS);
        int enq = 0;
        for (;;) {
            static const int perPoll = getenv("VSLAM_BA_STEPS_PER_POLL") ? std::max(1, atoi(getenv("VSLAM_BA_STEPS_PER_POLL"))) : 4;
            for (int b = 0; b < perPoll; b++) VS_CHECK(step(enq + b == 0));
            enq += perPoll;
            VS_HIP(hipMemcpyAsync(h_ctlOut, D.ctl, CTL_DOUBLES * sizeof(double), hipMemcpyDeviceToHost, stream));
            VS_HIP(vslam::stream_wait_blocking(stream));
            if (co[CI_STATE] == BA_DONE) break;
            if (enq > 400) { set_error("local BA: LM did not terminate"); return VSLAM_ERR_INVALID; }
        }
        D.poseCur = d_poseS.p + (size_t)co[CI_SEL] * K; D.lmCur = d_lmS.p + (size_t)co[CI_SEL] * 3 * L;
        R->report[ps].iterations = co[CI_ITER];
        R->report[ps].inner_iterations = co[CI_INNER];
        R->report[ps].initial_error = h_ctlOut[CTL_INIT_ERR];
        R->report[ps].final_error = h_ctlOut[CTL_ERROR];
        R->report[ps].lambda = h_ctlOut[CTL_LAMBDA];
        R->n_residuals = nfStat; R->n_landmarks = lpStat; R->n_free_kf = F; R->sum_k2 = k2Stat;
        R->rounds = (ps == 0 ? 0 : R->rounds) + co[CI_ROUNDS];

        if (comm) {
            const int tc = g_baTimer.begin("ba_allreduce");
            if (L) {
                VS_HIP(d_lmDiff.alloc((size_t)3 * L));
                hipLaunchKernelGGL(k_ba_lm_diff, dim3((3 * L + 255) / 256), dim3(256), 0, stream, 3 * L, D.lmCur, p_lm0, d_lmDiff.p, 0);
                VS_CHECK(comm_allreduce(comm, d_lmDiff.p, (size_t)3 * L, stream));
                hipLaunchKernelGGL(k_ba_lm_apply, dim3((3 * L + 255) / 256), dim3(256), 0, stream, 3 * L, D.lmCur, p_lm0, d_lmDiff.p);
            }
            double st[4] = {(double)nfStat, (double)lpStat, (double)k2Stat, 0.0};
            VS_HIP(hipMemcpyAsync(d_sums.p + 4, st, sizeof(st), hipMemcpyHostToDevice, stream));
            VS_CHECK(comm_allreduce(comm, d_sums.p + 4, 3, stream));
            VS_HIP(hipMemcpyAsync(st, d_sums.p + 4, sizeof(st), hipMemcpyDeviceToHost, stream));
            VS_HIP(hipStreamSynchronize(stream));
            R->n_residuals = (int64_t)llround(st[0]); R->n_landmarks = (int64_t)llround(st[1]); R->sum_k2 = (int64_t)llround(st[2]);
            g_baTimer.end(tc);
        }
        BHS("lm");
        BaChi C{};
        C.NP = NP; C.pairKf = p_pairKf; C.pairLm = p_pairLm; C.pairFlags = p_pairFlags; C.pairUv = p_pairUv;
        C.pairOct = p_pairOct; C.kfLocal = p_kfLocal; C.kfPresent = A.dev(h_kfPresent); C.lmPresent = A.dev(h_lmPresent);
        C.pose = D.poseCur; C.lm = D.lmCur; C.wrong = d_wrong.p;
        for (int l = 0; l < P->n_levels; l++) C.thr[l] = (float)((double)7.815f * (double)P->sigma_factor[l]);
        C.fx = D.fx; C.fy = D.fy; C.cx = D.cx; C.cy = D.cy; C.b = D.b;
        int t = g_baTimer.begin("ba_chi2");
        if (NP) hipLaunchKernelGGL(k_ba_chi2, dim3((NP + 255) / 256), dim3(256), 0, stream, C);
        g_baTimer.end(t);
        VS_HIP(hipGetLastError());
        if (NP) VS_HIP(hipMemcpyAsync(ws->h_wrong, d_wrong.p, NP, hipMemcpyDeviceToHost, stream));
        if (ps == 1) {
            VS_HIP(hipMemcpyAsync(poseOut, D.poseCur, K * sizeof(DPose), hipMemcpyDeviceToHost, stream));
            if (L) VS_HIP(hipMemcpyAsync(lmOut, D.lmCur, (size_t)3 * L * sizeof(double), hipMemcpyDeviceToHost, stream));
            resultFetched = true;
        }
        VS_HIP(hipStreamSynchronize(stream));
        if (NP) memcpy(wrong.data(), ws->h_wrong, NP);
        if (ps == 0 && R->pair_wrong_pass1 && NP) memcpy(R->pair_wrong_pass1, wrong.data(), NP);
        poseFinal = D.poseCur;
        lmFinal = D.lmCur;
        return VSLAM_OK;
        };
        VS_CHECK(run_lm(pass, NF, Lp, sumK2));

        static const bool maskEnv = !getenv("VSLAM_BA_NO_MASK");
        if (pass == 0 && maskEnv && g_baMask) {
            std::vector<uint8_t> kfP2(K, 0), lmP2(devOrder ? 0 : L, 0);
            long long NF2 = 0, Lp2dev = 0, k2dev = 0;
            if (devOrder) {
                const size_t zInts = (size_t)L + K + ((size_t)L + 3) / 4;
                VS_HIP(hipMemsetAsync(ws->d_ord1.p, 0, zInts * sizeof(int), stream));
                const int pairBlocks = std::max(1, std::min((NP + 255) / 256, 8 * nCU));
                hipLaunchKernelGGL(k_ord_count, dim3(pairBlocks), dim3(256), 0, stream, O);
                hipLaunchKernelGGL(k_ord_scan_lm, dim3(1), dim3(1024), 0, stream, O);
                if (Lp > 0) hipLaunchKernelGGL(k_ord_k2_masked, dim3((Lp + 255) / 256), dim3(256), 0, stream, O, Lp);
                VS_HIP(hipGetLastError());
// ... 78 lines not shown
    if (L) memcpy(R->lm_xyz, lmOut, (size_t)3 * L * sizeof(double));
    if (NP) memcpy(R->pair_wrong, wrong.data(), NP);
    return VSLAM_OK;
}

static std::atomic<long long> g_bbsNs[12], g_bbsCalls{0}, g_bbsPolls{0};
static const char* g_bbsName[12] = {"check+count", "arena fill", "tables+upload", "lm pass 1", "chi2 1", "second-pass prep", "lm pass 2", "chi2 2 + fetch", "results", nullptr, nullptr, nullptr};

struct BaPlanKnobs { bool schur2, back2, sharedW; int s2Waves, b2Waves, schurWaves, lmBlocks, s2Layout; };
static BaPlanKnobs ba_plan_knobs() {
    static const bool s2Env = !(getenv("VSLAM_BA_SCHUR2") && atoi(getenv("VSLAM_BA_SCHUR2")) == 0);
    static const bool b2Env = !(getenv("VSLAM_BA_BACK2") && atoi(getenv("VSLAM_BA_BACK2")) == 0);
    BaPlanKnobs k;
    k.schur2 = s2Env; k.back2 = b2Env;
    k.sharedW = getenv("VSLAM_BA_SCHUR_SHARED") ? atoi(getenv("VSLAM_BA_SCHUR_SHARED")) != 0 : true;
    k.schurWaves = getenv("VSLAM_BA_SCHUR_WAVES_B") ? atoi(getenv("VSLAM_BA_SCHUR_WAVES_B")) : 0;
    k.lmBlocks = getenv("VSLAM_BA_LMBLOCKS") ? atoi(getenv("VSLAM_BA_LMBLOCKS")) : 0;
    k.s2Waves = getenv("VSLAM_BA_SCHUR2_WAVES") ? atoi(getenv("VSLAM_BA_SCHUR2_WAVES")) : 8;
    k.b2Waves = getenv("VSLAM_BA_BACK2_WAVES") ? atoi(getenv("VSLAM_BA_BACK2_WAVES")) : 4;
    k.s2Layout = getenv("VSLAM_BA_SCHUR2_LAYOUT") ? std::max(0, std::min((int)BA2_PACKED, atoi(getenv("VSLAM_BA_SCHUR2_LAYOUT")))) : (int)BA2_PACKED;
    return k;
}
static inline int ba_batch_solve_kind(int n, bool useMfma) { return (n <= 64 && useMfma) ? BA_SOLVE_MFMA64 : n <= BA_WAVE_N ? BA_SOLVE_WAVE : BA_SOLVE_MFMA; }
static inline bool ba_batch_single(const vslam_ba_lane_shape& s, bool useMfma) {
    return s.own_rig || s.n_free_kf > BA_LDS_MAX_F || s.n_free_kf <= 0 || s.n_factors <= 0 || s.n_pairs <= 0 || (!useMfma && 6 * s.n_free_kf > BA_WAVE_N);
}
static void ba_batch_plan(const vslam_ba_batch_shape& S, const BaPlanKnobs& kn, vslam_ba_batch_plan& p) {
    p = vslam_ba_batch_plan{};
    const int NB = std::max(1, std::min((int)BA_MAX_NB, (int)S.lookahead));
    const bool useMfma = S.solver == 0;
    p.status = VSLAM_OK; p.lookahead = NB;
    int maxSlots = 1, maxFac = 1, fMax = 0, lpMax = 0, NL = 0;
    for (int i = 0; i < S.n_lanes; i++) {
        const vslam_ba_lane_shape& s = S.lanes[i];
        if (ba_batch_single(s, useMfma)) { p.n_single++; continue; }
        NL++;
        maxSlots = std::max(maxSlots, (int)s.max_slots); maxFac = std::max(maxFac, (int)s.max_factors);
        fMax = std::max(fMax, (int)s.n_free_kf); lpMax = std::max(lpMax, (int)s.n_points);
        p.solve_kinds |= 1 << ba_batch_solve_kind(6 * s.n_free_kf, useMfma);
    }
    p.n_batch = NL; p.f_max = fMax; p.max_slots = maxSlots; p.max_factors = maxFac; p.lp_max = lpMax;
    if (NL == 0) { p.solve_kinds = 0; return; }
    const int nCU = 256, nMax = 6 * fMax;
    const size_t sysMax = (size_t)nMax * nMax + nMax;
    constexpr int SCHUR_LPW = 64 / BA_LPL_SCHUR, BACK_LPW = 64 / BA_LPL_BACK;
    auto stage_lds = [&](int nw) { return (size_t)nw * SCHUR_LPW * 2 * maxSlots * 18 * sizeof(double) + (size_t)nw * SCHUR_LPW * maxSlots * sizeof(int) + 16; };
    auto schur_lds = [&](int nw, int copies) { return copies * sysMax * sizeof(double) + stage_lds(nw); };
    int sharedW = 0, schurWaves = BA_SCHUR_WAVES;
    if (NB > 1 && kn.sharedW) for (int nw : {16, 12, 8, 6, 4, 2}) if (schur_lds(nw, NB) <= 150 * 1024) { sharedW = 1; schurWaves = nw; break; }
    if (!sharedW) { if (kn.schurWaves) schurWaves = kn.schurWaves; while (schurWaves > 2 && schur_lds(schurWaves, 1) > 150 * 1024) schurWaves /= 2; }
    const size_t schurLds = schur_lds(schurWaves, sharedW ? NB : 1);
    const int schurUnits = schurWaves * SCHUR_LPW;
    int lmBlocks = std::max(1, std::min((lpMax + schurUnits - 1) / schurUnits, kn.lmBlocks ? kn.lmBlocks : std::max(16, 2 * nCU / NL)));
    const size_t s2StageB = (size_t)ba2_stage_doubles(maxFac, maxSlots) * sizeof(double);
    int s2Waves = std::max(2, std::min(16, kn.s2Waves));
    while (s2Waves > 2 && sysMax * sizeof(double) + s2Waves * s2StageB > 156 * 1024) s2Waves /= 2;
    const size_t s2Lds = sysMax * sizeof(double) + (size_t)s2Waves * s2StageB;
    const bool useSchur2 = kn.schur2 && fMax <= BA2_MAX_F && maxSlots <= BA2_MAX_F && s2Lds <= 156 * 1024;
    if (useSchur2) lmBlocks = std::max(1, std::min((lpMax + 2 * s2Waves - 1) / (2 * s2Waves), kn.lmBlocks ? kn.lmBlocks : std::max(4, (16 / s2Waves) * nCU / NL)));
    int b2Waves = std::max(1, std::min(8, kn.b2Waves));
    while (b2Waves > 1 && (size_t)b2Waves * s2StageB > BA_DYN_LDS_MAX) b2Waves /= 2;
    const size_t b2Lds = (size_t)b2Waves * s2StageB;
    const bool useBack2 = useSchur2 && kn.back2 && b2Lds <= BA_DYN_LDS_MAX;
    int backWaves = BA_SCHUR_WAVES / BACK_LPW;
    auto back_lds = [&](int nw) { return (size_t)nw * BACK_LPW * maxSlots * 18 * sizeof(double) + (size_t)nw * BACK_LPW * maxSlots * sizeof(int) + 16; };
    while (backWaves > 1 && back_lds(backWaves) > 150 * 1024) backWaves /= 2;
    p.schur_kernel = useSchur2 ? VSLAM_BA_KERNEL_SCHUR2 : VSLAM_BA_KERNEL_SCHUR;
    p.schur_waves = useSchur2 ? s2Waves : schurWaves;
    p.schur_shared_w = useSchur2 ? 0 : sharedW;
    p.schur_blocks = lmBlocks;
    p.schur_lds = (int)(useSchur2 ? (size_t)ba2_sys_doubles(nMax, kn.s2Layout) * sizeof(double) + (size_t)s2Waves * s2StageB : schurLds);
    p.back_kernel = useBack2 ? VSLAM_BA_KERNEL_BACK2 : VSLAM_BA_KERNEL_BACK;
    if (useBack2) {
        p.back_waves = b2Waves; p.back_shared = 1; p.back_lds = (int)b2Lds;
        p.back_blocks = std::max(1, std::min((lpMax + 2 * b2Waves - 1) / (2 * b2Waves), std::max(8, (16 / b2Waves) * nCU / NL)));
    } else {
        p.back_waves = backWaves; p.back_shared = NB > 1 ? 1 : 0; p.back_lds = (int)back_lds(backWaves);
        p.back_blocks = std::max(1, std::min((lpMax + backWaves * BACK_LPW - 1) / (backWaves * BACK_LPW), std::max(16, 2 * nCU / NL)));
    }
    p.solve_lds = (p.solve_kinds & (1 << BA_SOLVE_MFMA)) ? (int)(((size_t)BA_MFMA_N * BA_MFMA_LD + 16 + BA_MFMA_N) * sizeof(double)) : 0;
    if (p.schur_lds > BA_DYN_LDS_MAX || p.back_lds > BA_DYN_LDS_MAX || p.solve_lds > BA_DYN_LDS_MAX) p.status = VSLAM_ERR_CAPACITY;
}
thread_local vslam_ba_batch_plan g_baLastPlan{};

static vslam_status ba_run_batch(const vslam_ba_problem* const* Ps, vslam_ba_result* const* Rs, int N, int device) {
    g_baLastPlan = vslam_ba_batch_plan{};
    if (N <= 0 || !Ps || !Rs) return VSLAM_ERR_INVALID;
    if (N == 1) { g_baLastPlan.n_single = 1; return ba_run(Ps[0], Rs[0], device, nullptr); }
    auto bbs_t = std::chrono::steady_clock::now();
    g_bbsCalls++;
    auto BBS = [&](int k) { const auto t_ = std::chrono::steady_clock::now(); g_bbsNs[k] += std::chrono::duration_cast<std::chrono::nanoseconds>(t_ - bbs_t).count(); bbs_t = t_; };
    int ndev = 0;
    if (hipGetDeviceCount(&ndev) != hipSuccess || ndev <= 0) { set_error("no HIP device available (no CPU fallback)"); return VSLAM_ERR_NO_DEVICE; }
    if (device < 0 || device >= ndev) return VSLAM_ERR_INVALID;
    VS_HIP(hipSetDevice(device));
    struct BatchWs {
        hipStream_t stream = nullptr; int device = -1;
        PinnedArena arena;
        DevBuf<uint8_t> d_mem;
        uint8_t* h_back = nullptr; size_t backCap = 0;
        BaPool pool;
        void release() {
            if (device < 0 || hipSetDevice(device) != hipSuccess) return;
            if (stream) { hipStreamSynchronize(stream); hipStreamDestroy(stream); }
            if (d_mem.p) hipFree(d_mem.p);
            if (arena.d) hipFree(arena.d);
            if (arena.h) hipHostFree(arena.h);
            if (h_back) hipHostFree(h_back);
        }
    };
    static thread_local std::unique_ptr<BatchWs> bws;
    static thread_local void (*prevRelease)() = nullptr;
    if (!bws || bws->device != device) {
        if (bws) bws->release();
        bws.reset(new BatchWs()); bws->device = device;
        VS_HIP(vslam::create_side_stream(&bws->stream));
        bws->pool.start(2);
        prevRelease = g_baRelease;
        g_baRelease = []() { if (bws) { bws->release(); bws.reset(); } if (prevRelease) { auto f = prevRelease; prevRelease = nullptr; f(); } g_baTimer.destroy(); };
    }
    BatchWs& W = *bws;
    hipStream_t stream = W.stream;
    g_baTimer.reset(); g_baTimer.stream = stream; g_baTimer.multi = true;

    static const int nbEnv = [] { const char* e = getenv("VSLAM_BA_LOOKAHEAD"); return e ? std::max(1, std::min((int)BA_MAX_NB, atoi(e))) : (int)BA_MAX_NB; }();
    const int NB = g_baLookahead > 0 ? std::min(g_baLookahead, (int)BA_MAX_NB) : nbEnv, nSlots = NB + 1;
    const bool useMfma = ba_use_mfma();
    const double relTol = 1e-5, absTol = 1e-5;
    static const int adaptEnv = [] { const char* e = getenv("VSLAM_BA_ADAPTIVE"); return e ? atoi(e) : -1; }();
    const bool adaptive = NB > 1 && (adaptEnv >= 0 ? adaptEnv != 0 : true);

    struct Lane {
        const vslam_ba_problem* P; vslam_ba_result* R; int K, L, NP;
        std::vector<DPose> pose0; BaHostTmp T; BaPassHost H; bool single = false, ownRig = false;
        std::vector<uint8_t> wrong;
        DPose* h_pose0; double* h_lm0; int *h_pairKf, *h_pairLm, *h_pairOct; uint8_t *h_pairFlags, *h_kfLocal; float* h_pairUv;
        DPose* d_poseS; double *d_lmS, *d_facJ, *d_dP, *d_dL, *d_S, *d_Sedge, *d_partial, *d_Spart, *d_sums, *d_Lg; int* d_flags; uint8_t* d_wrong;
        double *d_outPose, *d_outLm;
        size_t oWrong, oOut;
        long long NF2 = 0, Lp2 = 0, k2 = 0;
        bool pass2 = false;
    };
    std::vector<Lane> lanes(N);
    auto lane_shape = [](const Lane& q) {
        vslam_ba_lane_shape s{};
        s.n_free_kf = q.H.F; s.n_points = q.H.Lp; s.n_factors = q.H.NF; s.n_edges = q.H.NE; s.n_pairs = q.NP;
        s.max_slots = q.H.maxSlots; s.max_factors = q.H.maxFac; s.own_rig = q.ownRig ? 1 : 0;
        return s;
    };
    std::vector<int> singles;
    for (int i = 0; i < N; i++) {
        Lane& q = lanes[i];
        const vslam_ba_problem* P = Ps[i]; vslam_ba_result* R = Rs[i];
        if (!P || !R || P->n_kf < 1 || P->n_lm < 0 || P->n_pairs < 0 || P->n_levels < 1 || P->n_levels > MAX_LEVELS ||
            !P->kf_pose_wc || !P->kf_id || !P->kf_fixed || !P->kf_local || !P->sigma_factor || !P->inv_sigma_factor ||
            !R->kf_pose_wc || !R->lm_xyz || !R->pair_wrong || (P->n_lm > 0 && !P->lm_xyz) ||
            (P->n_pairs > 0 && (!P->pair_kf || !P->pair_lm || !P->pair_flags || !P->pair_uv || !P->pair_octave))) {
            set_error("vslam_local_ba_batch: invalid problem %d", i);
            return VSLAM_ERR_INVALID;
        }
        q.P = P; q.R = R; q.K = P->n_kf; q.L = P->n_lm; q.NP = P->n_pairs;
        for (int p = 0; p < q.NP; p++)
            if (P->pair_kf[p] < 0 || P->pair_kf[p] >= q.K || P->pair_lm[p] < 0 || P->pair_lm[p] >= q.L ||
                P->pair_octave[2 * p] < 0 || P->pair_octave[2 * p] >= P->n_levels || P->pair_octave[2 * p + 1] < 0 ||
                P->pair_octave[2 * p + 1] >= P->n_levels) { set_error("vslam_local_ba_batch: pair index out of range (problem %d)", i); return VSLAM_ERR_INVALID; }
        q.ownRig = P->n_levels != Ps[0]->n_levels;
        q.wrong.assign(std::max(q.NP, 1), 0);
        q.pose0.resize(q.K);
        for (int k = 0; k < q.K; k++) pose_from_rm16(P->kf_pose_wc + 16 * (size_t)k, q.pose0[k]);
// ... 82 lines not shown
    size_t dBytes = 0;
    auto dtake = [&](size_t bytes) { const size_t at = dBytes; dBytes = (dBytes + std::max<size_t>(bytes, 8) + 255) & ~(size_t)255; return at; };
    struct Off { size_t flags, sedge, poseS, lmS, facJ, dP, dL, S, partial, spart, sums, Lg, wrong, outPose, outLm; };
    std::vector<Off> off(NL);
    for (int a = 0; a < NL; a++) { const Lane& q = lanes[act[a]]; off[a].flags = dtake(16 * sizeof(int)); off[a].sedge = dtake(((size_t)q.H.n * q.H.n + q.H.n) * nSlots * 8); }
    const size_t zeroBytes = dBytes;
    size_t wrongBase = 0, wrongEnd = 0, outBase = 0, outEnd = 0;
    wrongBase = dBytes;
    for (int a = 0; a < NL; a++) off[a].wrong = dtake(lanes[act[a]].NP);
    wrongEnd = dBytes;
    outBase = dBytes;
    for (int a = 0; a < NL; a++) { const Lane& q = lanes[act[a]]; off[a].outPose = dtake((size_t)q.K * sizeof(DPose)); off[a].outLm = dtake((size_t)3 * q.L * 8); }
    outEnd = dBytes;
    for (int a = 0; a < NL; a++) {
        const Lane& q = lanes[act[a]];
        const BaPassHost& H = q.H;
        const size_t sysStride = (size_t)H.n * H.n + 2 * H.n + 8;
        off[a].poseS = dtake((size_t)nSlots * q.K * sizeof(DPose)); off[a].lmS = dtake((size_t)nSlots * 3 * q.L * 8);
        off[a].facJ = dtake((size_t)20 * H.NF * nSlots * 8); off[a].dP = dtake((size_t)NB * H.n * 8); off[a].dL = dtake((size_t)NB * 3 * H.Lp * 8);
        off[a].S = dtake(sysStride * NB * 8); off[a].partial = dtake(((size_t)2 * obsBlocks + 2 * (size_t)std::max(H.NE, 1)) * NB * 8);
        off[a].spart = dtake(part_doubles(H.n) * lmBlocks * NB * 8); off[a].sums = dtake(32 * 8);
        off[a].Lg = (H.n > 64 || !useMfma) && H.n > BA_WAVE_N ? dtake((size_t)BA_MFMA_N * BA_MFMA_N * NB * 8) : 0;
    }
    VS_HIP(W.d_mem.alloc(dBytes));
    uint8_t* const dm = W.d_mem.p;
    const size_t oBackCtl = 0, oBackWrong = ((size_t)CTL_DOUBLES * 8 * NL + 255) & ~(size_t)255, oBackOut = oBackWrong + (wrongEnd - wrongBase);
    const size_t backBytes = oBackOut + (outEnd - outBase);
    if (backBytes > W.backCap) {
        VS_HIP(hipStreamSynchronize(stream));
        if (W.h_back) hipHostFree(W.h_back);
        W.backCap = 2 * backBytes + 4096;
        VS_HIP(hipHostMalloc((void**)&W.h_back, W.backCap, hipHostMallocDefault));
    }
    for (int a = 0; a < NL; a++) {
        Lane& q = lanes[act[a]];
        const BaPassHost& H = q.H;
        const vslam_ba_problem* P = q.P;
        const Off& o = off[a];
        q.d_flags = (int*)(dm + o.flags); q.d_Sedge = (double*)(dm + o.sedge); q.d_poseS = (DPose*)(dm + o.poseS); q.d_lmS = (double*)(dm + o.lmS);
        q.d_facJ = (double*)(dm + o.facJ); q.d_dP = (double*)(dm + o.dP); q.d_dL = (double*)(dm + o.dL); q.d_S = (double*)(dm + o.S);
        q.d_partial = (double*)(dm + o.partial); q.d_Spart = (double*)(dm + o.spart); q.d_sums = (double*)(dm + o.sums);
        q.d_Lg = o.Lg ? (double*)(dm + o.Lg) : nullptr; q.oWrong = oBackWrong + (o.wrong - wrongBase); q.oOut = oBackOut + (o.outPose - outBase);
        q.d_wrong = W.h_back + q.oWrong; q.d_outPose = (double*)(W.h_back + q.oOut);
        q.d_outLm = (double*)(W.h_back + q.oOut + (o.outLm - o.outPose));
        BaDev D{};
        const int n = H.n, K = q.K, L = q.L;
        D.NF = H.NF; D.Lp = H.Lp; D.F = H.F; D.K = K; D.NE = H.NE; D.n = n;
        D.facKf = A.dev(H.h_facKf); D.facFi = A.dev(H.h_facFi); D.facLp = A.dev(H.h_facLp); D.facLm = A.dev(H.h_facLm);
        D.facZ = A.dev(H.h_facZ); D.facIs = A.dev(H.h_facIs); D.facRight = A.dev(H.h_facRight); D.facJ = q.d_facJ;
        D.lpStart = A.dev(H.h_lpStart); D.lpSlotStart = A.dev(H.h_lpSlotStart); D.slotStart = A.dev(H.h_slotStart); D.slotFi = A.dev(H.h_slotFi);
        D.lpOrig = A.dev(H.h_lpOrig); D.poseCur = q.d_poseS; D.poseTrial = q.d_poseS + K; D.fidx = A.dev(H.h_fidx);
        D.lmCur = q.d_lmS; D.lmTrial = q.d_lmS + (size_t)3 * L; D.edges = A.dev(H.h_edges);
        D.S = q.d_S; D.rhs = q.d_S + (size_t)n * n; D.Sedge = q.d_Sedge; D.dP = q.d_dP; D.dL = q.d_dL; D.sums = q.d_sums; D.flags = q.d_flags;
        D.fx = P->rig.fx; D.fy = P->rig.fy; D.cx = P->rig.cx; D.cy = P->rig.cy; D.b = (double)P->rig.baseline;
        D.ctl = A.dev(H.h_ctl);
        D.NB = NB; D.specLin = 1; D.adaptive = adaptive ? 1 : 0;
        D.poseBase = q.d_poseS; D.lmBase = q.d_lmS; D.lmStride = (size_t)3 * L;
        D.facJBase = q.d_facJ; D.facJStride = (size_t)20 * H.NF; D.SedgeBase = q.d_Sedge; D.edgesBase = A.dev(H.h_edges);
        D.sysStride = (size_t)n * n + 2 * n + 8; D.dLStride = (size_t)3 * H.Lp;
        D.partialStride = (size_t)2 * obsBlocks + 2 * (size_t)std::max(H.NE, 1); D.partial = q.d_partial;
        D.spartStride = part_doubles(n) * lmBlocks; D.Spart = q.d_Spart;
        D.solveKind = ba_batch_solve_kind(n, useMfma);
        D.Lg = q.d_Lg;
        D.ctlHost = (double*)(W.h_back + oBackCtl) + (size_t)CTL_DOUBLES * a;
        *H.h_D = D;
        BaLaneAux X{};
        X.C.NP = q.NP; X.C.pairKf = A.dev(q.h_pairKf); X.C.pairLm = A.dev(q.h_pairLm); X.C.pairFlags = A.dev(q.h_pairFlags); X.C.pairUv = A.dev(q.h_pairUv);
        X.C.pairOct = A.dev(q.h_pairOct); X.C.kfLocal = A.dev(q.h_kfLocal); X.C.kfPresent = A.dev(H.h_kfPresent); X.C.lmPresent = A.dev(H.h_lmPresent);
        X.C.wrong = q.d_wrong;
        for (int l = 0; l < P->n_levels; l++) X.C.thr[l] = (float)((double)7.815f * (double)P->sigma_factor[l]);
        X.C.fx = D.fx; X.C.fy = D.fy; X.C.cx = D.cx; X.C.cy = D.cy; X.C.b = D.b;
        X.NF = H.NF; X.facPair = A.dev(H.h_facPair); X.facIs = A.dev(H.h_facIs);
        X.nPose = K * (int)(sizeof(DPose) / sizeof(double)); X.nLm = 3 * L; X.pose0 = (const double*)A.dev(q.h_pose0); X.lm0 = A.dev(q.h_lm0);
        X.outPose = q.d_outPose; X.outLm = q.d_outLm;
        h_aux[a] = X;
    }
    const BaDev* const dTab = A.dev(h_tab);
    const BaLaneAux* const dAux = A.dev(h_aux);
    VS_HIP(A.upload(stream));
    VS_HIP(hipMemsetAsync(dm, 0, zeroBytes, stream));
    const int valBlocks = std::max(1, std::min((valMax + 255) / 256, 64));
    hipLaunchKernelGGL(k_ba_init_slots_b, dim3(valBlocks, NL), dim3(256), 0, stream, dTab, dAux);

    auto step = [&](bool first) -> vslam_status {
        int t = -1;
        if (first) {
            t = g_baTimer.begin("ba_linearize");
            hipLaunchKernelGGL(k_ba_factors<0>, dim3(facBlocks, 1, NL), dim3(256), 0, stream, dTab, obsBlocks, 1, relTol, absTol);
            g_baTimer.end(t);
        }
        t = g_baTimer.begin("ba_schur");
        if (useSchur2 && s2Layout == BA2_PACKED) hipLaunchKernelGGL(k_ba_schur2, dim3(lmBlocks, NB, NL), dim3(64 * plan.schur_waves), plan.schur_lds, stream, dTab, maxSlots, maxFac);
        else if (useSchur2) hipLaunchKernelGGL(k_ba_schur2_rm, dim3(lmBlocks, NB, NL), dim3(64 * plan.schur_waves), plan.schur_lds, stream, dTab, maxSlots, maxFac, s2Layout);
        else hipLaunchKernelGGL(k_ba_schur, dim3(lmBlocks, plan.schur_shared_w ? 1 : NB, NL), dim3(64 * plan.schur_waves), plan.schur_lds, stream, dTab, maxSlots, plan.schur_shared_w);
        g_baTimer.end(t);
        t = g_baTimer.begin("ba_solve");
        hipLaunchKernelGGL(k_ba_reduce, dim3((reduceSlots + 31) / 32, NB, NL), dim3(256), 0, stream, dTab, lmBlocks, packedS ? 1 : 0);
        if (anyMfma64) hipLaunchKernelGGL(k_ba_solve_mfma64, dim3(NB, 1, NL), dim3(64), 0, stream, dTab);
        if (anyWave) hipLaunchKernelGGL(k_ba_solve_wave, dim3(NB, 1, NL), dim3(64), 0, stream, dTab);
        if (anyMfma) hipLaunchKernelGGL(k_ba_solve_mfma, dim3(NB, 1, NL), dim3(64 * BA_MFMA_NW), plan.solve_lds, stream, dTab, (double*)nullptr);
        g_baTimer.end(t);
        t = g_baTimer.begin("ba_back");
        if (useBack2) hipLaunchKernelGGL(k_ba_back2, dim3(plan.back_blocks, 1, NL), dim3(64 * plan.back_waves), plan.back_lds, stream, dTab, maxSlots, maxFac);
        else hipLaunchKernelGGL(k_ba_back, dim3(plan.back_blocks, plan.back_shared ? 1 : NB, NL), dim3(64 * plan.back_waves), plan.back_lds, stream, dTab, maxSlots, plan.back_shared);
        g_baTimer.end(t);
        t = g_baTimer.begin("ba_eval");
        hipLaunchKernelGGL(k_ba_factors<1>, dim3(facBlocks, NB, NL), dim3(256), 0, stream, dTab, obsBlocks, 1, relTol, absTol);
        g_baTimer.end(t);
        VS_HIP(hipGetLastError());
        return VSLAM_OK;
    };
    double* const b_ctl = (double*)(W.h_back + oBackCtl);
    memcpy(b_ctl, h_ctlAll, (size_t)CTL_DOUBLES * 8 * NL);
    auto lm_loop = [&](int first) -> vslam_status {
        static const int perPollEnv = getenv("VSLAM_BA_STEPS_PER_POLL") ? std::max(1, atoi(getenv("VSLAM_BA_STEPS_PER_POLL"))) : 0;
        int enq = 0, polls = 0;
        for (;;) {
            const int batch = perPollEnv ? perPollEnv : (enq == 0 ? first : 2);
            for (int b = 0; b < batch; b++) VS_CHECK(step(enq + b == 0));
            enq += batch;
            static const bool mirrorOff = getenv("VSLAM_BA_CTL_MIRROR") && atoi(getenv("VSLAM_BA_CTL_MIRROR")) == 0;
            if (mirrorOff || ++polls > 4) VS_HIP(hipMemcpyAsync(b_ctl, A.dev(h_ctlAll), (size_t)CTL_DOUBLES * 8 * NL, hipMemcpyDeviceToHost, stream));
            VS_HIP(vslam::stream_wait_blocking(stream));
            g_bbsPolls++;
            bool all = true;
            for (int a = 0; a < NL; a++) all &= ((const int*)(b_ctl + (size_t)CTL_DOUBLES * a + CTL_INTS))[CI_STATE] == BA_DONE;
            if (all) return VSLAM_OK;
            if (enq > 400) {
                (void)hipMemcpy(b_ctl, A.dev(h_ctlAll), (size_t)CTL_DOUBLES * 8 * NL, hipMemcpyDeviceToHost);
                for (int a = 0; a < NL; a++) {
                    const double* c = b_ctl + (size_t)CTL_DOUBLES * a;
                    const int* ci = (const int*)(c + CTL_INTS);
                    if (ci[CI_STATE] == BA_DONE) continue;
                    int fl[8] = {0};
                    (void)hipMemcpy(fl, lanes[act[a]].d_flags, sizeof(fl), hipMemcpyDeviceToHost);
                    set_error("local BA batch: LM did not terminate (lane %d of %d: state %d sel %d iter %d inner %d maxit %d first %d nact %d rounds %d lambda %g error %g cur %g; "
                              "F %d NF %d Lp %d NE %d; flags %d %d %d %d | %d %d %d %d; obsBlocks %d neMax %d)", a, NL, ci[CI_STATE], ci[CI_SEL], ci[CI_ITER], ci[CI_INNER], ci[CI_MAXIT], ci[CI_FIRST], ci[CI_NACT], ci[CI_ROUNDS],
                              c[CTL_LAMBDA], c[CTL_ERROR], c[CTL_CUR], lanes[act[a]].H.F, lanes[act[a]].H.NF, lanes[act[a]].H.Lp, lanes[act[a]].H.NE,
                              fl[0], fl[1], fl[2], fl[3], fl[4], fl[5], fl[6], fl[7], obsBlocks, neMax);
                    return VSLAM_ERR_INVALID;
                }
                set_error("local BA batch: LM did not terminate (every lane done on the device: the host's copy lagged)");
                return VSLAM_ERR_INVALID;
            }
        }
    };
    auto report = [&](int ps) {
        for (int a = 0; a < NL; a++) {
            Lane& q = lanes[act[a]];
            if (ps == 1 && !q.pass2) continue;
            const double* c = b_ctl + (size_t)CTL_DOUBLES * a;
            const int* ci = (const int*)(c + CTL_INTS);
            vslam_ba_result* R = q.R;
            R->report[ps].iterations = ci[CI_ITER]; R->report[ps].inner_iterations = ci[CI_INNER];
            R->report[ps].initial_error = c[CTL_INIT_ERR]; R->report[ps].final_error = c[CTL_ERROR]; R->report[ps].lambda = c[CTL_LAMBDA];
            R->n_free_kf = q.H.F;
            R->rounds = (ps == 0 ? 0 : R->rounds) + ci[CI_ROUNDS];
            if (ps == 0) { R->n_residuals = q.H.NF; R->n_landmarks = q.H.Lp; R->sum_k2 = q.H.sumK2; }
            else { R->n_residuals = q.NF2; R->n_landmarks = q.Lp2; R->sum_k2 = q.k2; }
        }
    };
    const int chiBlocks = std::max(1, (std::max(npMax, valMax) + 255) / 256);
    auto chi2 = [&](int gather) -> vslam_status {
        const int t = g_baTimer.begin("ba_chi2");
        hipLaunchKernelGGL(k_ba_chi2_b, dim3(chiBlocks, NL), dim3(256), 0, stream, dTab, dAux, gather);
        g_baTimer.end(t);
        VS_HIP(hipGetLastError());
        VS_HIP(vslam::stream_wait_blocking(stream));
        return VSLAM_OK;
    };
    BBS(2);
    VS_CHECK(lm_loop(5));
    report(0);
    BBS(3);
    VS_CHECK(chi2(0));
    BBS(4);
    std::vector<int> redo;
    W.pool.run(NL, [&](int a) {
        Lane& q = lanes[act[a]];
        const vslam_ba_problem* P = q.P;
        const BaPassHost& H = q.H;
        memcpy(q.wrong.data(), W.h_back + q.oWrong, q.NP);
        if (q.R->pair_wrong_pass1) memcpy(q.R->pair_wrong_pass1, q.wrong.data(), q.NP);
        std::vector<uint8_t> kfP2(q.K, 0), lmP2(std::max(q.L, 1), 0);
        long long NF2 = 0;
        for (int p = 0; p < q.NP; p++) {
            if (q.wrong[p]) continue;
            const int fl = P->pair_flags[p] & 3;
            if (!fl) continue;
            kfP2[P->pair_kf[p]] = 1; lmP2[P->pair_lm[p]] = 1; NF2 += (fl & 1) + (fl >> 1);
        }
        bool same = g_baMask != 0;
        for (int k = 0; k < q.K && same; k++) if (kfP2[k] != q.T.kfPresent[k]) same = false;
        int* ci = (int*)(H.h_ctl + CTL_INTS);
        if (!same) { q.pass2 = false; ci[CI_STATE] = BA_DONE; ci[CI_FIRST] = 0; return; }
        long long Lp2 = 0, k2 = 0;
        for (int l = 0; l < q.L; l++) Lp2 += lmP2[l];
        for (int lp = 0; lp < H.Lp; lp++) {
            int ns = 0, last = -2;
            for (int f = H.h_lpStart[lp]; f < H.h_lpStart[lp + 1]; f++) {
                if (q.wrong[H.h_facPair[f]]) continue;
                const int fi = H.h_facFi[f];
                if (fi >= 0 && fi != last) { last = fi; ns++; }
            }
            k2 += (long long)ns * ns;
        }
        q.NF2 = NF2; q.Lp2 = Lp2; q.k2 = k2; q.pass2 = true;
        for (int k = 0; k < q.K; k++) H.h_kfPresent[k] = kfP2[k];
        for (int l = 0; l < q.L; l++) H.h_lmPresent[l] = lmP2[l];
        ba_init_ctl(H.h_ctl, 1, adaptive ? 1 : NB);
    });
    for (int a = 0; a < NL; a++) if (!lanes[act[a]].pass2) redo.push_back(act[a]);
    BBS(5);
    if ((int)redo.size() < NL) {
        VS_HIP(hipMemcpyAsync(A.dev(h_ctlAll), h_ctlAll, (size_t)CTL_DOUBLES * 8 * NL, hipMemcpyHostToDevice, stream));
        VS_HIP(hipMemcpyAsync(A.dev(h_present), h_present, presentBytes, hipMemcpyHostToDevice, stream));
        memcpy(b_ctl, h_ctlAll, (size_t)CTL_DOUBLES * 8 * NL);
        hipLaunchKernelGGL(k_ba_second_pass_b, dim3(std::max(1, std::min((std::max(nfMax, valMax) + 255) / 256, 64)), NL), dim3(256), 0, stream, dTab, dAux);
        VS_CHECK(lm_loop(6));
        report(1);
        BBS(6);
        VS_CHECK(chi2(1));
        BBS(7);
    }
    for (int a = 0; a < NL; a++) {
        Lane& q = lanes[act[a]];
        if (!q.pass2) continue;
        const DPose* po = (const DPose*)(W.h_back + q.oOut);
        const double* lo = (const double*)(W.h_back + q.oOut + (((size_t)q.K * sizeof(DPose) + 255) & ~(size_t)255));
        for (int k = 0; k < q.K; k++) pose_to_rm16(po[k], q.R->kf_pose_wc + 16 * (size_t)k);
        if (q.L) memcpy(q.R->lm_xyz, lo, (size_t)3 * q.L * sizeof(double));
        if (q.NP) memcpy(q.R->pair_wrong, W.h_back + q.oWrong, q.NP);
    }
    BBS(8);
    for (int i : redo) VS_CHECK(ba_run(Ps[i], Rs[i], device, nullptr));
    return run_singles();
}

namespace vslam {
void ba_host_profile_print() {
#ifndef VSLAM_HOST_STAMPS
    if (const long long nb = g_bbsCalls.load()) {
        fprintf(stderr, "  vslam_local_ba_batch host sections (us per cohort, %lld cohorts, %.1f polls each):", nb, (double)g_bbsPolls.load() / (double)nb);
        for (int i = 0; i < 12 && g_bbsName[i]; i++) fprintf(stderr, " %s %.1f |", g_bbsName[i], 1e-3 * (double)g_bbsNs[i].load() / (double)nb);
        fprintf(stderr, "\n");
    }
    const long long n = g_bhsCalls.load();
    if (!n) return;
    fprintf(stderr, "  vslam_local_ba host sections (us per call, %lld calls):", n);
    for (int i = 0; i < 16; i++) if (g_bhsName[i] || g_bhsNs[i].load()) fprintf(stderr, " %s %.1f |", g_bhsName[i] ? g_bhsName[i] : "other", 1e-3 * (double)g_bhsNs[i].load() / (double)n);
    fprintf(stderr, "\n");
#endif
}
}

extern "C" {

vslam_status vslam_local_ba(const vslam_ba_problem* problem, vslam_ba_result* result, int32_t device,
                            const vslam_comm* comm) {
    return ba_run(problem, result, device, comm);
}

vslam_status vslam_local_ba_batch(const vslam_ba_problem* const* problems, vslam_ba_result* const* results, int32_t n, int32_t device) {
    return ba_run_batch(problems, results, n, device);
}

vslam_status vslam_local_ba_batch_plan(const vslam_ba_batch_shape* shape, vslam_ba_batch_plan* plan) {
    if (!shape || !plan || shape->n_lanes < 0 || (shape->n_lanes > 0 && !shape->lanes) || shape->lookahead < 1 || shape->lookahead > BA_MAX_NB ||
        shape->solver < 0 || shape->solver > 1) return VSLAM_ERR_INVALID;
    ba_batch_plan(*shape, ba_plan_knobs(), *plan);
    return VSLAM_OK;
}

vslam_status vslam_local_ba_last_batch_plan(vslam_ba_batch_plan* plan) {
    if (!plan) return VSLAM_ERR_INVALID;
    *plan = g_baLastPlan;
    return VSLAM_OK;
}

vslam_status vslam_local_ba_timings(const char** names, float* ms, int32_t cap, int32_t* n_out) {
    if (!n_out) return VSLAM_ERR_INVALID;
    const char* nm[64];
    float tv[64];
    int n = g_baTimer.read(nm, tv, cap < 64 ? cap : 64);
    for (int i = 0; i < n; i++) { if (names) names[i] = nm[i]; if (ms) ms[i] = tv[i]; }
    static const char* const cntName[][2] = {{"ba_linearize", "ba_linearize#n"}, {"ba_schur", "ba_schur#n"}, {"ba_solve", "ba_solve#n"},
                                             {"ba_back", "ba_back#n"}, {"ba_eval", "ba_eval#n"}, {"ba_chi2", "ba_chi2#n"}, {"ba_allreduce", "ba_allreduce#n"}};
    const int base = n;
    for (int i = 0; i < base && n < cap; i++)
        for (const auto& c : cntName)
            if (!strcmp(nm[i], c[0])) {
                int k = 0;
                for (size_t q = 0; q < g_baTimer.used; q++) if (!strcmp(g_baTimer.items[q].name, c[0])) k++;
                if (names) names[n] = c[1];
                if (ms) ms[n] = (float)k;
                n++;
                break;
            }
    *n_out = n;
    return VSLAM_OK;
}

vslam_status vslam_local_ba_set_lookahead(int32_t candidates, int32_t speculative_linearize, int32_t mask_second_pass) {
    if (candidates > BA_MAX_NB) return VSLAM_ERR_INVALID;
    g_baLookahead = candidates > 0 ? candidates : -1;
    g_baSpecLin = speculative_linearize < 0 ? -1 : (speculative_linearize ? 1 : 0);
    g_baMask = mask_second_pass != 0 ? 1 : 0;
    return VSLAM_OK;
}

vslam_status vslam_local_ba_set_solver(int32_t kind) {
    if (kind < -1 || kind > 1) return VSLAM_ERR_INVALID;
    g_baSolver = kind;
    return VSLAM_OK;
}

vslam_status vslam_local_ba_set_timing(int32_t on) {
    g_baTimer.enabled = on != 0;
    return VSLAM_OK;
}
int32_t vslam_local_ba_get_timing(void) { return g_baTimer.enabled ? 1 : 0; }

}

namespace vslam {
vslam_status refresh_depth_enqueue(const float* kf_close_th, int n_kf, const double* kf_pose_wc, int n_lm, const double* lm_xyz,
                                   const uint8_t* lm_outlier, int n_pairs, const int* pair_kf, const int* pair_lm, const uint8_t* pair_wrong,
                                   const float* cur_depth, int device, RefreshTicket* out) {
    if (n_pairs <= 0 || n_kf < 1 || !out || !kf_close_th) return VSLAM_ERR_INVALID;
    if (const char* e = getenv("VSLAM_REFRESH_FORCE_CAPACITY")) if (atoi(e) != 0) return VSLAM_ERR_CAPACITY;
    VS_HIP(hipSetDevice(device));
    DevPool* pool = thread_pool(device);
    if (!pool) { set_error("no device pool"); return VSLAM_ERR_HIP; }
    size_t off = 0;
    auto take = [&](size_t bytes) { const size_t o = off; off = (off + bytes + 255) & ~(size_t)255; return o; };
    const size_t oT = take(n_kf * sizeof(DPose)), oTh = take(n_kf * sizeof(float)), oLm = take((size_t)3 * std::max(n_lm, 1) * sizeof(double)),
                 oO = take(std::max(n_lm, 1)), oKf = take(n_pairs * sizeof(int)), oL = take(n_pairs * sizeof(int)), oW = take(n_pairs),
                 oCur = take(n_pairs * sizeof(float)), oD = take(n_pairs * sizeof(float)), oC = take(n_pairs), oU = take(n_pairs);
    uint8_t* st = pool->stage(off);
    if (!st) return VSLAM_ERR_CAPACITY;
    DPose* Tcw = (DPose*)(st + oT);
    for (int k = 0; k < n_kf; k++) { DPose T; pose_from_rm16(kf_pose_wc + 16 * (size_t)k, T); pose_inverse(T, Tcw[k]); }
    memcpy(st + oTh, kf_close_th, n_kf * sizeof(float));
    if (n_lm) { memcpy(st + oLm, lm_xyz, (size_t)3 * n_lm * sizeof(double)); memcpy(st + oO, lm_outlier, n_lm); }
    memcpy(st + oKf, pair_kf, n_pairs * sizeof(int)); memcpy(st + oL, pair_lm, n_pairs * sizeof(int));
    memcpy(st + oW, pair_wrong, n_pairs); memcpy(st + oCur, cur_depth, n_pairs * sizeof(float));
    hipLaunchKernelGGL(k_ba_refresh_depth, dim3((n_pairs + 255) / 256), dim3(256), 0, pool->stream, n_pairs, (const int*)(st + oKf),
                       (const int*)(st + oL), (const uint8_t*)(st + oW), (const uint8_t*)(st + oO), (const float*)(st + oCur),
                       (const DPose*)(st + oT), (const double*)(st + oLm), (const float*)(st + oTh), 0.f, (float*)(st + oD), st + oC, st + oU);
    VS_HIP(hipGetLastError());
    out->dep = (const float*)(st + oD); out->clo = st + oC; out->up = st + oU;
    return VSLAM_OK;
}
// ... 122 lines not shown
```

gtsam-vslam_amd/vslam_capi.py:

```python
import ctypes as C
import os
import subprocess
import numpy as np

_HERE = os.path.dirname(os.path.abspath(__file__))
LIB_PATH = os.path.join(_HERE, "libvslam_hip.so")
_LIB = None

KP_DTYPE = np.dtype([("x", "<f4"), ("y", "<f4"), ("size", "<f4"), ("angle", "<f4"),
                     ("response", "<f4"), ("octave", "<i4"), ("class_id", "<i4")])

OK, ERR_INVALID, ERR_NO_DEVICE, ERR_HIP, ERR_CAPACITY, ERR_COMM = range(6)


class FeParams(C.Structure):
    _fields_ = [("n_features", C.c_int32), ("n_levels", C.c_int32), ("scale", C.c_float),
                ("edge_threshold", C.c_int32), ("patch_size", C.c_int32),
                ("max_fast_threshold", C.c_int32), ("min_fast_threshold", C.c_int32)]


class VslamError(RuntimeError):
    def __init__(self, status, msg):
        super().__init__("vslam status %d: %s" % (status, msg))
        self.status = status
# ... 491 lines not shown
    poct = np.ascontiguousarray(prob["pair_oct"], np.int32).reshape(-1, 2)
    sf = np.ascontiguousarray(sigma_factor, np.float32); isf = np.ascontiguousarray(inv_sigma_factor, np.float32)
    P = BaProblem()
    P.rig = make_rig(rig)
    P.n_levels = len(sf); P.sigma_factor = _p(sf); P.inv_sigma_factor = _p(isf)
    P.n_kf = len(kfPose); P.kf_pose_wc = _p(kfPose); P.kf_id = _p(kfId); P.kf_fixed = _p(kfFixed); P.kf_local = _p(kfLocal)
    P.n_lm = len(lm); P.lm_xyz = _p(lm) if len(lm) else None
    P.n_pairs = len(pk)
    if len(pk):
        P.pair_kf, P.pair_lm, P.pair_flags, P.pair_uv, P.pair_octave = _p(pk), _p(pl), _p(pf), _p(puv), _p(poct)
    kfOut = np.zeros_like(kfPose); lmOut = np.zeros((max(len(lm), 1), 3))
    wrong = np.zeros(max(len(pk), 1), np.uint8); wrong1 = np.zeros(max(len(pk), 1), np.uint8)
    R = BaResult()
    R.kf_pose_wc, R.lm_xyz, R.pair_wrong, R.pair_wrong_pass1 = _p(kfOut), _p(lmOut), _p(wrong), _p(wrong1)

    def read():
        reps = [dict(iterations=R.report[s].iterations, inner=R.report[s].inner_iterations,
                     initialError=R.report[s].initial_error, finalError=R.report[s].final_error, lam=R.report[s].lam)
                for s in range(2)]
        return dict(kf_pose=kfOut.reshape(-1, 4, 4), lm=lmOut[:len(lm)], pair_wrong=wrong[:len(pk)],
                    pair_wrong1=wrong1[:len(pk)], reports=reps, residuals=R.n_residuals, landmarks=R.n_landmarks,
                    free_kf=R.n_free_kf, sum_k2=R.sum_k2, rounds=R.rounds)
    keep = dict(arrays=[kfPose, kfId, kfFixed, kfLocal, lm, pk, pl, pf, puv, poct, sf, isf, kfOut, lmOut, wrong, wrong1], read=read)
    return P, R, keep


def local_ba(rig, sigma_factor, inv_sigma_factor, prob, device=0, comm=None):
    P, R, keep = ba_problem_structs(rig, sigma_factor, inv_sigma_factor, prob)
    _chk(lib().vslam_local_ba(C.byref(P), C.byref(R), device, comm.h if comm is not None else None))
    return keep["read"]()


def local_ba_batch(rig, sigma_factor, inv_sigma_factor, probs, device=0):
    n = len(probs)
    rigs = list(rig) if isinstance(rig, (list, tuple)) else [rig] * n
    built = [ba_problem_structs(rigs[i], sigma_factor, inv_sigma_factor, pr) for i, pr in enumerate(probs)]
    PP = (C.POINTER(BaProblem) * n)(*[C.pointer(b[0]) for b in built])
    RR = (C.POINTER(BaResult) * n)(*[C.pointer(b[1]) for b in built])
    _chk(lib().vslam_local_ba_batch(PP, RR, n, int(device)))
    return [b[2]["read"]() for b in built]


class BaLaneShape(C.Structure):
    _fields_ = [(f, C.c_int32) for f in ("n_free_kf", "n_points", "n_factors", "n_edges", "n_pairs", "max_slots", "max_factors", "own_rig")]


class BaBatchShape(C.Structure):
    _fields_ = [("n_lanes", C.c_int32), ("lanes", C.POINTER(BaLaneShape)), ("lookahead", C.c_int32), ("solver", C.c_int32)]


class BaBatchPlan(C.Structure):
    _fields_ = [(f, C.c_int32) for f in ("status", "n_batch", "n_single", "lookahead", "f_max", "max_slots", "max_factors", "lp_max",
                                         "schur_kernel", "schur_waves", "schur_shared_w", "schur_blocks", "schur_lds",
                                         "back_kernel", "back_waves", "back_shared", "back_blocks", "back_lds", "solve_kinds", "solve_lds")]


BA_KERNELS = {0: None, 1: "schur", 2: "schur2", 3: "back", 4: "back2"}
BA_SOLVES = {1: "mfma64", 2: "wave", 4: "mfma"}


def _plan_dict(p):
    d = {f: int(getattr(p, f)) for f, _ in BaBatchPlan._fields_}
    d["schur_kernel"] = BA_KERNELS[d["schur_kernel"]]
    d["back_kernel"] = BA_KERNELS[d["back_kernel"]]
    d["solves"] = {name for bit, name in BA_SOLVES.items() if d["solve_kinds"] & bit}
    return d


def local_ba_batch_plan(lanes, lookahead=4, solver=0):
    arr = (BaLaneShape * max(len(lanes), 1))()
    for i, ln in enumerate(lanes):
        for k, v in ln.items():
            setattr(arr[i], k, int(v))
    S = BaBatchShape(len(lanes), arr, int(lookahead), int(solver))
    P = BaBatchPlan()
    _chk(lib().vslam_local_ba_batch_plan(C.byref(S), C.byref(P)))
    return _plan_dict(P)


def local_ba_last_batch_plan():
    P = BaBatchPlan()
    _chk(lib().vslam_local_ba_last_batch_plan(C.byref(P)))
    return _plan_dict(P)


def local_ba_timings():
    names = (C.c_char_p * 32)()
    ms = (C.c_float * 32)()
    n = C.c_int32()
    _chk(lib().vslam_local_ba_timings(names, ms, 32, C.byref(n)))
    return {names[i].decode(): float(ms[i]) for i in range(n.value)}


def ba_refresh_depth(rig, kf_pose_wc, lm_xyz, lm_outlier, pair_kf, pair_lm, pair_wrong, cur_depth, device=0):
    T = np.ascontiguousarray(kf_pose_wc, np.float64).reshape(-1, 16)
    lm = np.ascontiguousarray(lm_xyz, np.float64).reshape(-1, 3); lo = np.ascontiguousarray(lm_outlier, np.uint8)
    pk = np.ascontiguousarray(pair_kf, np.int32); pl = np.ascontiguousarray(pair_lm, np.int32)
    pw = np.ascontiguousarray(pair_wrong, np.uint8); cd = np.ascontiguousarray(cur_depth, np.float32)
    n = len(pk)
    d = np.zeros(max(n, 1), np.float32); c = np.zeros(max(n, 1), np.uint8); u = np.zeros(max(n, 1), np.uint8)
    r = make_rig(rig)
    _chk(lib().vslam_ba_refresh_depth(C.byref(r), len(T), _p(T), len(lm), _p(lm), _p(lo), n, _p(pk), _p(pl), _p(pw), _p(cd), int(device),
                                      _p(d), _p(c), _p(u)))
    return d[:n], c[:n], u[:n]


def ba_refresh_depth_merged(rigs, n_kfs, kf_pose_wc, lm_xyz, lm_outlier, pair_kf, pair_lm, pair_wrong, cur_depth, device=0):
    T = np.ascontiguousarray(kf_pose_wc, np.float64).reshape(-1, 16)
    lm = np.ascontiguousarray(lm_xyz, np.float64).reshape(-1, 3); lo = np.ascontiguousarray(lm_outlier, np.uint8)
    pk = np.ascontiguousarray(pair_kf, np.int32); pl = np.ascontiguousarray(pair_lm, np.int32)
    pw = np.ascontiguousarray(pair_wrong, np.uint8); cd = np.ascontiguousarray(cur_depth, np.float32)
    n = len(pk)
    d = np.zeros(max(n, 1), np.float32); c = np.zeros(max(n, 1), np.uint8); u = np.zeros(max(n, 1), np.uint8)
    rg = (Rig * len(rigs))(*[make_rig(r) for r in rigs])
    nk = np.ascontiguousarray(n_kfs, np.int32)
    assert len(nk) == len(rigs) and int(nk.sum()) == len(T)
    _chk(lib().vslam_ba_refresh_depth_merged(rg, _p(nk), len(rigs), _p(T), len(lm), _p(lm), _p(lo), n, _p(pk), _p(pl), _p(pw), _p(cd),
                                             int(device), _p(d), _p(c), _p(u)))
    return d[:n], c[:n], u[:n]


def local_ba_set_timing(on):
    _chk(lib().vslam_local_ba_set_timing(int(bool(on))))


def local_ba_set_solver(kind=-1):
    _chk(lib().vslam_local_ba_set_solver(int(kind)))


def local_ba_set_lookahead(candidates=0, speculative_linearize=-1, mask_second_pass=1):
    _chk(lib().vslam_local_ba_set_lookahead(int(candidates), int(speculative_linearize), int(mask_second_pass)))


class TrackReport(C.Structure):
    _fields_ = [("n_map_points", C.c_int32), ("n_active", C.c_int32), ("rounds", C.c_int32),
                ("n_inliers", C.c_int32), ("n_stereo", C.c_int32), ("lm_iterations", C.c_int32),
                ("last_radius", C.c_float)]


def tracker_init_map(matcher, T_wc):
    T = np.ascontiguousarray(T_wc, np.float64)
    _chk(matcher.L.vslam_tracker_init_map(matcher.h, _p(T)))


def tracker_track(matcher, T_wc_pred, frame_number):
    T = np.ascontiguousarray(T_wc_pred, np.float64)
    out = np.zeros((4, 4), np.float64)
    rep = TrackReport()
    _chk(matcher.L.vslam_tracker_track(matcher.h, _p(T), int(frame_number), _p(out), C.byref(rep)))
    return out, {f[0]: getattr(rep, f[0]) for f in TrackReport._fields_}


def tracker_fetch(matcher, cap=65536):
    mt = np.zeros((cap, 2), np.int32); out = np.zeros(cap, np.uint8); act = np.zeros(cap, np.int32)
    n = C.c_int32()
    _chk(matcher.L.vslam_tracker_fetch(matcher.h, _p(mt), _p(out), _p(act), cap, C.byref(n)))
    return mt[:n.value].copy(), out[:n.value].copy(), act[:n.value].copy()


class Comm:
    def __init__(self, handle):
        self.h = handle

    def close(self):
        if self.h:
            lib().vslam_comm_destroy(self.h)
# ... 1169 lines not shown
```

include/vslam_hip.h:

```cpp
#ifndef VSLAM_HIP_H
#define VSLAM_HIP_H

#include <stddef.h>
#include <stdint.h>

#ifdef __cplusplus
extern "C" {
#endif

typedef enum vslam_status {
    VSLAM_OK = 0,
    VSLAM_ERR_INVALID = 1,
    VSLAM_ERR_NO_DEVICE = 2,
    VSLAM_ERR_HIP = 3,
    VSLAM_ERR_CAPACITY = 4,
    VSLAM_ERR_COMM = 5
} vslam_status;

const char* vslam_last_error(void);
int vslam_device_count(void);

typedef struct vslam_keypoint {
    float x, y;
    float size;
// ... 259 lines not shown
                                    uint8_t* updated_out);
vslam_status vslam_ba_refresh_depth_merged(const vslam_rig* rigs, const int32_t* req_n_kf, int32_t n_req, const double* kf_pose_wc,
                                           int32_t n_lm, const double* lm_xyz, const uint8_t* lm_outlier, int32_t n_pairs,
                                           const int32_t* pair_kf, const int32_t* pair_lm, const uint8_t* pair_wrong,
                                           const float* cur_depth, int32_t device, float* depth_out, uint8_t* close_out,
                                           uint8_t* updated_out);

typedef struct {
    vslam_rig rig;
    int32_t n_levels;
    const float* inv_sigma_factor;
    int64_t numb;
    const double* key_pose;
    const double* ref_pose;
    const double* cur_pose_inv;
    int32_t n_left, n_right;
    const vslam_keypoint* kps_left; const vslam_keypoint* kps_right;
    const int32_t* slot_lm_l; const int32_t* slot_lm_r;
    int32_t n_lm;
    double* lm_xyz;
    const int64_t* lm_kdx;
    const uint8_t* lm_outlier;
} vslam_kf_update_problem;

vslam_status vslam_keyframe_update_pose(const vslam_kf_update_problem* problem, int32_t device, uint8_t* drop_l,
                                        uint8_t* drop_r, double* pose_out);

vslam_status vslam_save_trajectory(const char* path_trajectory, const char* path_positions, int32_t n_frames,
                                   const uint8_t* is_keyframe, const double* pose_or_ref);

typedef struct vslam_comm vslam_comm;
vslam_status vslam_comm_unique_id(uint8_t id_out[128]);
vslam_status vslam_comm_create_rccl(const uint8_t id[128], int32_t rank, int32_t world, int32_t device,
                                    vslam_comm** out);
vslam_status vslam_comm_create_local(int32_t world, vslam_comm** out_array );
typedef int (*vslam_allreduce_fn)(void* ctx, double* host_buf, size_t n);
vslam_status vslam_comm_create_callback(int32_t rank, int32_t world, int32_t device, vslam_allreduce_fn allreduce, void* ctx,
                                        vslam_comm** out);
void vslam_comm_destroy(vslam_comm* comm);

vslam_status vslam_local_ba_batch(const vslam_ba_problem* const* problems, vslam_ba_result* const* results, int32_t n, int32_t device);

typedef struct vslam_ba_lane_shape {
    int32_t n_free_kf;
    int32_t n_points;
    int32_t n_factors;
    int32_t n_edges;
    int32_t n_pairs;
    int32_t max_slots;
    int32_t max_factors;
    int32_t own_rig;
} vslam_ba_lane_shape;

typedef struct vslam_ba_batch_shape {
    int32_t n_lanes;
    const vslam_ba_lane_shape* lanes;
    int32_t lookahead;
    int32_t solver;
} vslam_ba_batch_shape;

enum {
    VSLAM_BA_KERNEL_NONE = 0,
    VSLAM_BA_KERNEL_SCHUR = 1,
    VSLAM_BA_KERNEL_SCHUR2 = 2,
    VSLAM_BA_KERNEL_BACK = 3,
    VSLAM_BA_KERNEL_BACK2 = 4
};
enum { VSLAM_BA_SOLVE_MFMA64 = 1, VSLAM_BA_SOLVE_WAVE = 2, VSLAM_BA_SOLVE_MFMA = 4 };

typedef struct vslam_ba_batch_plan {
    int32_t status;
    int32_t n_batch;
    int32_t n_single;
    int32_t lookahead;
    int32_t f_max, max_slots, max_factors, lp_max;
    int32_t schur_kernel, schur_waves, schur_shared_w, schur_blocks, schur_lds;
    int32_t back_kernel, back_waves, back_shared, back_blocks, back_lds;
    int32_t solve_kinds;
    int32_t solve_lds;
} vslam_ba_batch_plan;

vslam_status vslam_local_ba_batch_plan(const vslam_ba_batch_shape* shape, vslam_ba_batch_plan* plan);
vslam_status vslam_local_ba_last_batch_plan(vslam_ba_batch_plan* plan);

vslam_status vslam_local_ba(const vslam_ba_problem* problem, vslam_ba_result* result, int32_t device,
                            const vslam_comm* comm);
vslam_status vslam_local_ba_timings(const char** names, float* ms, int32_t cap, int32_t* n_out);
vslam_status vslam_local_ba_set_timing(int32_t on);
int32_t vslam_local_ba_get_timing(void);
vslam_status vslam_local_ba_set_lookahead(int32_t candidates, int32_t speculative_linearize, int32_t mask_second_pass);
vslam_status vslam_local_ba_set_solver(int32_t kind);

size_t vslam_kf_keys_bytes(int32_t n_left, int32_t n_right);

typedef struct {
    const double* T_wc;
    int64_t id;
    int32_t n_left, n_right;
    const vslam_keypoint* kps_l; const uint8_t* desc_l;
    const vslam_keypoint* kps_r; const uint8_t* desc_r;
    const int32_t* right_idxs; const int32_t* left_idxs;
    const int32_t* unmatched_f; const int32_t* unmatched_fr;
    const void* device_keys;
    const float* estimated_depth; const uint8_t* close_flags;
} vslam_kf_view;
vslam_status vslam_kf_keys_upload(const vslam_kf_view* view, int32_t device, void* device_block);

typedef struct {
    vslam_rig rig;
    int32_t n_levels;
    const float* scale_pyramid;
    const float* sigma_factor;
    float log_scale;
    int32_t n_kf;
    const vslam_kf_view* kfs;
    const float* estimated_depth;
    const uint8_t* has_mp;
    const double* mp_xyz;
    const uint8_t* mp_desc;
} vslam_new_points_problem;

typedef struct {
    int32_t capacity;
    int32_t n_candidates;
    int32_t* cand_left; int32_t* cand_right;
    uint8_t* accepted;
    double* xyz;
    int32_t* n_obs;
    int32_t* obs;
} vslam_new_points_result;

vslam_status vslam_find_new_points(const vslam_new_points_problem* problem, vslam_new_points_result* result,
                                   int32_t device);
vslam_status vslam_find_new_points_batch(const vslam_new_points_problem* const* problems, vslam_new_points_result* const* results,
                                         int32_t n, int32_t device);

typedef struct {
    vslam_rig rig;
    int32_t n_levels;
    const float* sigma_factor;
    int32_t n_kf;
    const double* kf_pose_wc;
    const int32_t* kf_id;
    int32_t n_points;
    const int32_t* n_views;
    const int32_t* view_kf;
    const float* view_xy;
    const int32_t* view_octave;
} vslam_mono_points_problem;

typedef struct {
    uint8_t* accepted;
    double* xyz;
    int32_t* n_obs;
    uint8_t* keep;
} vslam_mono_points_result;

vslam_status vslam_mono_new_points(const vslam_mono_points_problem* problem, vslam_mono_points_result* result,
                                   int32_t device);

vslam_status vslam_calc_descriptors(const uint8_t* descs, const int32_t* start, int32_t n_mp, int32_t device,
                                    int32_t* best_out);

typedef struct vslam_track_report {
    int32_t n_map_points;
    int32_t n_active;
// ... 276 lines not shown
```

Before: 29320.

## Compact batched BA grids to live lanes and loop candidates inside blocks

Batched local BA kernels now take a bitmask of lanes that have not converged, built on the host from the mirrored control block, and size the grid z-dimension to the live count. Each block maps its z index to a real lane by popcount. Schur2 and reduce also loop over LM candidates inside one block instead of launching one y-slice per candidate. The aim is to stop launching blocks for finished lanes and unused candidates, at the cost of some per-block lane lookup and a possibly stale live mask from the last host poll. Work counters are added to the API.

```diff
diff --git a/gtsam-vslam_amd/csrc/ba.hip b/gtsam-vslam_amd/csrc/ba.hip
--- a/gtsam-vslam_amd/csrc/ba.hip
+++ b/gtsam-vslam_amd/csrc/ba.hip
@@ -81,6 +81,35 @@
     return true;
 }
 
+constexpr int BA_LIVE_WORDS = 8, BA_LIVE_BITS = 32 * BA_LIVE_WORDS;
+struct BaLive { unsigned w[BA_LIVE_WORDS]; int full; };
+__device__ __forceinline__ unsigned ba_live_lane(const BaLive& live) {
+    if (live.full) return blockIdx.z;
+    int k = (int)blockIdx.z;
+    unsigned m = 0, base = 0;
+    bool found = false;
+#pragma unroll
+    for (int i = 0; i < BA_LIVE_WORDS; i++) {
+        const unsigned w = live.w[i];
+        const int c = __builtin_popcount(w);
+        if (!found && k < c) { m = w; base = 32u * i; found = true; }
+        if (!found) k -= c;
+    }
+    for (; k > 0; k--) m &= m - 1;
+    return base + (m ? __builtin_ctz(m) : 0);
+}
+static inline BaLive ba_live_all() { BaLive l{}; l.full = 1; return l; }
+
+__device__ __forceinline__ int ba_tid() {
+    int t = threadIdx.x;
+    asm volatile("" : "+v"(t));
+    return t;
+}
+__device__ __forceinline__ const BaDev* ba_lane_block(const BaDev* tab, unsigned lane) {
+    asm volatile("" : "+s"(tab));
+    return lane_entry(tab, lane);
+}
+
 constexpr int BA_SCHUR_WAVES = 16;
 constexpr int BA_LDS_MAX_F = 20;
 constexpr int BA_LDS_BYTES = 160 * 1024, BA_STATIC_LDS_RESERVE = 1024, BA_DYN_LDS_MAX = BA_LDS_BYTES - BA_STATIC_LDS_RESERVE;
@@ -292,8 +321,8 @@
 }
 
 template <int MODE>
-__global__ __launch_bounds__(256) void k_ba_factors(const BaDev* __restrict__ tab, int obsBlocks, int fuseCtl, double relTol, double absTol) {
-    BaDev D = *lane_entry(tab, blockIdx.z);
+__global__ __launch_bounds__(256) void k_ba_factors(const BaDev* __restrict__ tab, BaLive live, int obsBlocks, int fuseCtl, double relTol, double absTol) {
+    BaDev D = *lane_entry(tab, ba_live_lane(live));
     __shared__ double red[8], out[2];
     __shared__ double sW[160];
     __shared__ int sLast;
@@ -464,8 +493,8 @@
     inv3sym(Hll, Hi);
 }
 
-__global__ __launch_bounds__(64 * BA_SCHUR_WAVES) void k_ba_schur(const BaDev* __restrict__ tab, int maxSlots, int sharedW) {
-    BaDev D = *lane_entry(tab, blockIdx.z);
+__global__ __launch_bounds__(64 * BA_SCHUR_WAVES) void k_ba_schur(const BaDev* __restrict__ tab, BaLive live, int maxSlots, int sharedW) {
+    BaDev D = *lane_entry(tab, ba_live_lane(live));
     constexpr bool LDS_S = true;
     extern __shared__ double sm[];
     double* const SBase = D.S;
@@ -663,18 +692,17 @@
 }
 
 template <bool PACKED>
-__device__ __forceinline__ void ba2_schur(const BaDev* __restrict__ tab, int maxSlots, int maxFac, int layout) {
-    BaDev D = *lane_entry(tab, blockIdx.z);
+__device__ __forceinline__ void ba2_schur_one(const BaDev& D, int maxSlots, int maxFac, int layout) {
     extern __shared__ double sm[];
-    if (!ba_enter(D, BA_TRY, blockIdx.y)) return;
     const int n = D.n, F = n / 6;
     constexpr bool packed = PACKED;
     const int ld = layout == BA2_ROWMAJOR1 ? n + 1 : n;
     const int sys = ba2_sys_doubles(n, layout);
     double* const Sloc = sm;
     double* const racc = Sloc + (packed ? ba_packed_rhs(F) : ld * n);
-    const int lane = threadIdx.x & 63;
-    const int unit = __builtin_amdgcn_readfirstlane(threadIdx.x >> 6), nu = blockDim.x >> 6, nt = blockDim.x;
+    const int tx = ba_tid();
+    const int lane = tx & 63;
+    const int unit = __builtin_amdgcn_readfirstlane(tx >> 6), nu = blockDim.x >> 6, nt = blockDim.x;
     const Ba2Region g = ba2_region(sm + sys + (size_t)unit * ba2_stage_doubles(maxFac, maxSlots), maxFac, maxSlots);
     double* const F_ = g.F; double* const W = g.W; double* const WH = g.WH;
     int* const ffi = g.ffi; int* const sfi = g.sfi;
@@ -682,7 +710,7 @@
     Ba2Roles R;
     R.init(lane);
     const int pf = lane / 6, pi = lane - pf * 6;
-    for (int i = threadIdx.x; i < sys; i += nt) Sloc[i] = 0;
+    for (int i = tx; i < sys; i += nt) Sloc[i] = 0;
     __syncthreads();
     for (int lp = blockIdx.x * nu + unit; lp < D.Lp; lp += gridDim.x * nu) {
         double h[9];
@@ -720,16 +748,26 @@
     const int part = ba2_part_doubles(n, layout);
     double* dst = D.Spart + (size_t)blockIdx.x * part;
     if (layout == BA2_ROWMAJOR1) {
-        for (int i = threadIdx.x; i < part; i += nt) dst[i] = Sloc[i + i / n];
+        for (int i = tx; i < part; i += nt) dst[i] = Sloc[i + i / n];
     } else {
-        for (int i = threadIdx.x; i < part; i += nt) dst[i] = Sloc[i];
-    }
-}
-__global__ __launch_bounds__(1024) void k_ba_schur2(const BaDev* __restrict__ tab, int maxSlots, int maxFac) { ba2_schur<true>(tab, maxSlots, maxFac, BA2_PACKED); }
-__global__ __launch_bounds__(1024) void k_ba_schur2_rm(const BaDev* __restrict__ tab, int maxSlots, int maxFac, int layout) { ba2_schur<false>(tab, maxSlots, maxFac, layout); }
-
-__global__ __launch_bounds__(512) void k_ba_back2(const BaDev* __restrict__ tab, int maxSlots, int maxFac) {
-    BaDev D = *lane_entry(tab, blockIdx.z);
+        for (int i = tx; i < part; i += nt) dst[i] = Sloc[i];
+    }
+}
+template <bool PACKED>
+__device__ __forceinline__ void ba2_schur(const BaDev* __restrict__ tab, const BaLive& live, int maxSlots, int maxFac, int layout) {
+    const unsigned ln = ba_live_lane(live);
+    for (int c = blockIdx.y; ; c += gridDim.y) {
+        BaDev D = *ba_lane_block(tab, ln);
+        if (!ba_enter(D, BA_TRY, c)) return;
+        ba2_schur_one<PACKED>(D, maxSlots, maxFac, layout);
+        __syncthreads();
+    }
+}
+__global__ __launch_bounds__(1024) void k_ba_schur2(const BaDev* __restrict__ tab, BaLive live, int maxSlots, int maxFac) { ba2_schur<true>(tab, live, maxSlots, maxFac, BA2_PACKED); }
+__global__ __launch_bounds__(1024) void k_ba_schur2_rm(const BaDev* __restrict__ tab, BaLive live, int maxSlots, int maxFac, int layout) { ba2_schur<false>(tab, live, maxSlots, maxFac, layout); }
+
+__global__ __launch_bounds__(512) void k_ba_back2(const BaDev* __restrict__ tab, BaLive live, int maxSlots, int maxFac) {
+    BaDev D = *lane_entry(tab, ba_live_lane(live));
     extern __shared__ double sm[];
     if (!ba_enter(D, BA_TRY, 0)) return;
     const int nc = D.nAct;
@@ -773,14 +811,12 @@
     }
 }
 
-__global__ __launch_bounds__(256) void k_ba_reduce(const BaDev* __restrict__ tab, int nPart, int packed) {
-    BaDev D = *lane_entry(tab, blockIdx.z);
-    __shared__ double sSl[8][33];
-    if (!ba_enter(D, BA_TRY, blockIdx.y)) return;
+__device__ __forceinline__ void ba_reduce_one(const BaDev& D, double (*sSl)[33], int nPart, int packed) {
     const int total = D.n * D.n + D.n, F = D.n / 6;
     const int nSum = packed ? ba_packed_doubles(F) : total;
     const int nSlots = packed ? ba_packed_reduce_slots(F) : total;
-    const int e = threadIdx.x & 31, y = threadIdx.x >> 5;
+    const int tx = ba_tid();
+    const int e = tx & 31, y = tx >> 5;
     const int i = blockIdx.x * 32 + e;
     double s = 0;
     if (i < nSum) {
@@ -799,15 +835,25 @@
     }
     sSl[y][e] = s;
     __syncthreads();
-    const int slot = blockIdx.x * 32 + threadIdx.x;
+    const int slot = blockIdx.x * 32 + tx;
     if (y == 0 && slot < nSlots) {
         const int io = packed ? ba_packed_reduce_entry(F, slot) : slot;
         if (io >= 0) {
             double t = D.Sedge[io];
-            for (int q = 0; q < 8; q++) t += sSl[q][threadIdx.x];
+            for (int q = 0; q < 8; q++) t += sSl[q][tx];
             if (D.specLin) D.Sedge2[io] = 0;
             if (io < D.n * D.n) D.S[io] = t; else D.rhs[io - D.n * D.n] = t;
         }
+    }
+}
+__global__ __launch_bounds__(256) void k_ba_reduce(const BaDev* __restrict__ tab, BaLive live, int nPart, int packed) {
+    const unsigned ln = ba_live_lane(live);
+    __shared__ double sSl[8][33];
+    for (int c = blockIdx.y; ; c += gridDim.y) {
+        BaDev D = *ba_lane_block(tab, ln);
+        if (!ba_enter(D, BA_TRY, c)) return;
+        ba_reduce_one(D, sSl, nPart, packed);
+        __syncthreads();
     }
 }
 
@@ -1144,12 +1190,9 @@
 }
 
 constexpr int BA_WAVE_N = 60;
-__global__ __launch_bounds__(64) void k_ba_solve_wave(const BaDev* __restrict__ tab) {
-    BaDev D = *lane_entry(tab, blockIdx.z);
+__device__ __forceinline__ void ba_solve_wave_one(const BaDev& D) {
     constexpr int N = BA_WAVE_N;
     __shared__ double Lt[N * (N + 1)];
-    if (D.solveKind != BA_SOLVE_WAVE) return;
-    if (!ba_enter(D, BA_TRY, blockIdx.x)) return;
     const double lambda = D.lambda;
     const int n = D.n, lane = threadIdx.x;
     const int r = lane < N ? lane : N - 1;
@@ -1219,19 +1262,22 @@
     BAW_STAMP(6)
     if (lane == 0) D.flags[FLAG_FAIL + D.cand] = bad ? 1 : 0;
 }
+__global__ __launch_bounds__(64) void k_ba_solve_wave(const BaDev* __restrict__ tab, BaLive live) {
+    BaDev D = *lane_entry(tab, ba_live_lane(live));
+    if (D.solveKind != BA_SOLVE_WAVE) return;
+    if (!ba_enter(D, BA_TRY, blockIdx.x)) return;
+    ba_solve_wave_one(D);
+}
 
 constexpr int BA_MFMA_N = 256, BA_MFMA_NB = BA_MFMA_N / 16, BA_MFMA_NW = 8, BA_MFMA_SLOTS = 17, BA_MFMA_LD = 17;
 typedef double ba_d4 __attribute__((ext_vector_type(4)));
 
-__global__ __launch_bounds__(64 * BA_MFMA_NW) void k_ba_solve_mfma(const BaDev* __restrict__ tab, double* __restrict__ Lg) {
-    BaDev D = *lane_entry(tab, blockIdx.z);
+__device__ __forceinline__ void ba_solve_mfma_one(const BaDev& D, double* __restrict__ Lg) {
     extern __shared__ double sm[];
     double* P = sm;
     double* sInv = P + BA_MFMA_N * BA_MFMA_LD;
     double* sB = sInv + 16;
     __shared__ int sBad;
-    if (D.solveKind != BA_SOLVE_MFMA) return;
-    if (!ba_enter(D, BA_TRY, blockIdx.x)) return;
     const double lambda = D.lambda;
     constexpr int N = BA_MFMA_N, NB = BA_MFMA_NB, LD = BA_MFMA_LD;
     if (D.Lg) Lg = D.Lg;
@@ -1383,15 +1429,18 @@
     }
     if (tid == 0) D.flags[FLAG_FAIL + D.cand] = fail ? 1 : 0;
 }
-
-__global__ __launch_bounds__(64) void k_ba_solve_mfma64(const BaDev* __restrict__ tab) {
-    BaDev D = *lane_entry(tab, blockIdx.z);
+__global__ __launch_bounds__(64 * BA_MFMA_NW) void k_ba_solve_mfma(const BaDev* __restrict__ tab, BaLive live, double* __restrict__ Lg) {
+    BaDev D = *lane_entry(tab, ba_live_lane(live));
+    if (D.solveKind != BA_SOLVE_MFMA) return;
+    if (!ba_enter(D, BA_TRY, blockIdx.x)) return;
+    ba_solve_mfma_one(D, Lg);
+}
+
+__device__ __forceinline__ void ba_solve_mfma64_one(const BaDev& D) {
     constexpr int N = 64, LDF = 65, LD = 17;
     __shared__ double Lf[N * LDF];
     __shared__ double P[N * LD];
     __shared__ double sInv[16], sB[N];
-    if (D.solveKind != BA_SOLVE_MFMA64) return;
-    if (!ba_enter(D, BA_TRY, blockIdx.x)) return;
     const double lambda = D.lambda;
     const int n = D.n, lane = threadIdx.x;
     auto fence = []() { asm volatile("s_waitcnt lgkmcnt(0)" ::: "memory"); };
@@ -1501,6 +1550,12 @@
         }
     }
     if (lane == 0) D.flags[FLAG_FAIL + D.cand] = bad ? 1 : 0;
+}
+__global__ __launch_bounds__(64) void k_ba_solve_mfma64(const BaDev* __restrict__ tab, BaLive live) {
+    BaDev D = *lane_entry(tab, ba_live_lane(live));
+    if (D.solveKind != BA_SOLVE_MFMA64) return;
+    if (!ba_enter(D, BA_TRY, blockIdx.x)) return;
+    ba_solve_mfma64_one(D);
 }
 
 constexpr int CH_B = 64, CH_LD = 65, CH_PLD = 17;
@@ -1732,8 +1787,8 @@
     }
 }
 
-__global__ __launch_bounds__(64 * BA_SCHUR_WAVES) void k_ba_back(const BaDev* __restrict__ tab, int maxSlots, int allCand) {
-    BaDev D = *lane_entry(tab, blockIdx.z);
+__global__ __launch_bounds__(64 * BA_SCHUR_WAVES) void k_ba_back(const BaDev* __restrict__ tab, BaLive live, int maxSlots, int allCand) {
+    BaDev D = *lane_entry(tab, ba_live_lane(live));
     extern __shared__ double sm[];
     const int c0 = allCand ? 0 : (int)blockIdx.y;
     if (!ba_enter(D, BA_TRY, c0)) return;
@@ -2937,11 +2992,12 @@
         const int facBlocks = (NF ? obsBlocks : 0) + std::max(NE, 1);
         const int nObs = NF ? obsBlocks : 0;
         VS_HIP(hipMemsetAsync(d_Sedge.p, 0, ((size_t)n * n + n) * sizeof(double), stream));
+        const BaLive oneLane = ba_live_all();
         auto step = [&](bool first) -> vslam_status {
             int t = -1;
             if (first || !specLin) {
                 t = g_baTimer.begin("ba_linearize");
-                hipLaunchKernelGGL(k_ba_factors<0>, dim3(facBlocks), dim3(256), 0, stream, dD, nObs, fuseCtl, relTol, absTol);
+                hipLaunchKernelGGL(k_ba_factors<0>, dim3(facBlocks), dim3(256), 0, stream, dD, oneLane, nObs, fuseCtl, relTol, absTol);
                 g_baTimer.end(t);
             }
             if (comm) {
@@ -2950,7 +3006,7 @@
             }
             t = g_baTimer.begin("ba_schur");
             if (n > 0) {
-                if (ldsS) hipLaunchKernelGGL(k_ba_schur, dim3(lmBlocks, sharedW ? 1 : NB), dim3(64 * schurWaves), schurLds, stream, dD, maxSlots, sharedW);
+                if (ldsS) hipLaunchKernelGGL(k_ba_schur, dim3(lmBlocks, sharedW ? 1 : NB), dim3(64 * schurWaves), schurLds, stream, dD, oneLane, maxSlots, sharedW);
                 else if (nWinWg) {
                     hipLaunchKernelGGL(k_ba_lm_prep, dim3(std::max(1, std::min((Lp + BA_SCHUR_WAVES - 1) / BA_SCHUR_WAVES, 4 * nCU))), dim3(64 * BA_SCHUR_WAVES),
                                        (size_t)BA_SCHUR_WAVES * maxSlots * sizeof(int), stream, dD, Wn, maxSlots);
@@ -2960,13 +3016,13 @@
             g_baTimer.end(t);
             t = g_baTimer.begin("ba_solve");
             if (n > 0) {
-                if (ldsS) hipLaunchKernelGGL(k_ba_reduce, dim3(((int)sysDoubles + 31) / 32, NB), dim3(256), 0, stream, dD, lmBlocks, 0);
+                if (ldsS) hipLaunchKernelGGL(k_ba_reduce, dim3(((int)sysDoubles + 31) / 32, NB), dim3(256), 0, stream, dD, oneLane, lmBlocks, 0);
                 else hipLaunchKernelGGL(k_ba_reduce_win, dim3(Wn.nWin, NB), dim3(256), 0, stream, dD, Wn);
             }
             if (comm && n > 0) { const int tc = g_baTimer.begin("ba_allreduce"); VS_CHECK(comm_allreduce(comm, d_S.p, sysStride * (NB - 1) + (size_t)n * n + n, stream)); g_baTimer.end(tc); }
-            if (n <= 64 && useMfma) hipLaunchKernelGGL(k_ba_solve_mfma64, dim3(NB), dim3(64), 0, stream, dD);
-            else if (n <= BA_WAVE_N) hipLaunchKernelGGL(k_ba_solve_wave, dim3(NB), dim3(64), 0, stream, dD);
-            else if (n <= BA_MFMA_N && useMfma) hipLaunchKernelGGL(k_ba_solve_mfma, dim3(NB), dim3(64 * BA_MFMA_NW), mfmaLds, stream, dD, d_Lg.p);
+            if (n <= 64 && useMfma) hipLaunchKernelGGL(k_ba_solve_mfma64, dim3(NB), dim3(64), 0, stream, dD, oneLane);
+            else if (n <= BA_WAVE_N) hipLaunchKernelGGL(k_ba_solve_wave, dim3(NB), dim3(64), 0, stream, dD, oneLane);
+            else if (n <= BA_MFMA_N && useMfma) hipLaunchKernelGGL(k_ba_solve_mfma, dim3(NB), dim3(64 * BA_MFMA_NW), mfmaLds, stream, dD, oneLane, d_Lg.p);
             else if (useChol) {
                 for (int J = 0; J < cholN / CH_B; J++)
                     hipLaunchKernelGGL(k_ba_chol_col, dim3(cholN / CH_B - J, NB), dim3(256), cholColLds, stream, dD, d_Lg.p, d_cholY.p, cholN, J, d_cholFail.p);
@@ -2975,10 +3031,10 @@
                                     solveLds ? solveLdsBytes : 64, stream, dD, solveLds ? 1 : 0, solveLds ? ldA : n);
             g_baTimer.end(t);
             t = g_baTimer.begin("ba_back");
-            if (Lp) hipLaunchKernelGGL(k_ba_back, dim3(backBlocks, sharedBack ? 1 : NB), dim3(64 * backWaves), backLds, stream, dD, maxSlots, sharedBack);
+            if (Lp) hipLaunchKernelGGL(k_ba_back, dim3(backBlocks, sharedBack ? 1 : NB), dim3(64 * backWaves), backLds, stream, dD, oneLane, maxSlots, sharedBack);
             g_baTimer.end(t);
             t = g_baTimer.begin("ba_eval");
-            hipLaunchKernelGGL(k_ba_factors<1>, dim3(facBlocks, NB), dim3(256), 0, stream, dD, nObs, fuseCtl, relTol, absTol);
+            hipLaunchKernelGGL(k_ba_factors<1>, dim3(facBlocks, NB), dim3(256), 0, stream, dD, oneLane, nObs, fuseCtl, relTol, absTol);
             g_baTimer.end(t);
             if (comm) {
                 const int tc = g_baTimer.begin("ba_allreduce"); VS_CHECK(comm_allreduce(comm, d_sums.p + SUMS_CAND, (size_t)2 * NB, stream)); g_baTimer.end(tc);
@@ -3223,9 +3279,11 @@
     if (p.schur_lds > BA_DYN_LDS_MAX || p.back_lds > BA_DYN_LDS_MAX || p.solve_lds > BA_DYN_LDS_MAX) p.status = VSLAM_ERR_CAPACITY;
 }
 thread_local vslam_ba_batch_plan g_baLastPlan{};
+thread_local vslam_ba_batch_work g_baLastWork{};
 
 static vslam_status ba_run_batch(const vslam_ba_problem* const* Ps, vslam_ba_result* const* Rs, int N, int device) {
     g_baLastPlan = vslam_ba_batch_plan{};
+    g_baLastWork = vslam_ba_batch_work{};
     if (N <= 0 || !Ps || !Rs) return VSLAM_ERR_INVALID;
     if (N == 1) { g_baLastPlan.n_single = 1; return ba_run(Ps[0], Rs[0], device, nullptr); }
     auto bbs_t = std::chrono::steady_clock::now();
@@ -3474,42 +3532,63 @@
     const int valBlocks = std::max(1, std::min((valMax + 255) / 256, 64));
     hipLaunchKernelGGL(k_ba_init_slots_b, dim3(valBlocks, NL), dim3(256), 0, stream, dTab, dAux);
 
-    auto step = [&](bool first) -> vslam_status {
+    const bool fullGrids = getenv("VSLAM_BA_FULL_GRIDS") && atoi(getenv("VSLAM_BA_FULL_GRIDS")) != 0;
+    const int liveCap = getenv("VSLAM_BA_LIVE_CAP") ? std::max(0, std::min((int)BA_LIVE_BITS, atoi(getenv("VSLAM_BA_LIVE_CAP")))) : (int)BA_LIVE_BITS;
+    const bool liveGrids = !fullGrids && NL <= liveCap;
+    const bool candLoop = !fullGrids && !(getenv("VSLAM_BA_CAND_LOOP") && atoi(getenv("VSLAM_BA_CAND_LOOP")) == 0);
+    const int candY = candLoop ? 1 : NB;
+    double* const b_ctl = (double*)(W.h_back + oBackCtl);
+    int nLive = NL;
+    auto live_set = [&]() {
+        BaLive live = ba_live_all();
+        nLive = NL;
+        if (!liveGrids) return live;
+        live = BaLive{};
+        nLive = 0;
+        for (int a = 0; a < NL; a++)
+            if (((const int*)(b_ctl + (size_t)CTL_DOUBLES * a + CTL_INTS))[CI_STATE] != BA_DONE) { live.w[a >> 5] |= 1u << (a & 31); nLive++; }
+        return live;
+    };
+    auto step = [&](bool first, const BaLive& live) -> vslam_status {
         int t = -1;
+        const int NZ = nLive;
+        if (NZ <= 0) return VSLAM_OK;
+        g_baLastWork.rounds_enqueued++; g_baLastWork.lane_slots += NZ;
         if (first) {
             t = g_baTimer.begin("ba_linearize");
-            hipLaunchKernelGGL(k_ba_factors<0>, dim3(facBlocks, 1, NL), dim3(256), 0, stream, dTab, obsBlocks, 1, relTol, absTol);
+            hipLaunchKernelGGL(k_ba_factors<0>, dim3(facBlocks, 1, NZ), dim3(256), 0, stream, dTab, live, obsBlocks, 1, relTol, absTol);
             g_baTimer.end(t);
         }
         t = g_baTimer.begin("ba_schur");
-        if (useSchur2 && s2Layout == BA2_PACKED) hipLaunchKernelGGL(k_ba_schur2, dim3(lmBlocks, NB, NL), dim3(64 * plan.schur_waves), plan.schur_lds, stream, dTab, maxSlots, maxFac);
-        else if (useSchur2) hipLaunchKernelGGL(k_ba_schur2_rm, dim3(lmBlocks, NB, NL), dim3(64 * plan.schur_waves), plan.schur_lds, stream, dTab, maxSlots, maxFac, s2Layout);
-        else hipLaunchKernelGGL(k_ba_schur, dim3(lmBlocks, plan.schur_shared_w ? 1 : NB, NL), dim3(64 * plan.schur_waves), plan.schur_lds, stream, dTab, maxSlots, plan.schur_shared_w);
+        if (useSchur2 && s2Layout == BA2_PACKED) hipLaunchKernelGGL(k_ba_schur2, dim3(lmBlocks, candY, NZ), dim3(64 * plan.schur_waves), plan.schur_lds, stream, dTab, live, maxSlots, maxFac);
+        else if (useSchur2) hipLaunchKernelGGL(k_ba_schur2_rm, dim3(lmBlocks, candY, NZ), dim3(64 * plan.schur_waves), plan.schur_lds, stream, dTab, live, maxSlots, maxFac, s2Layout);
+        else hipLaunchKernelGGL(k_ba_schur, dim3(lmBlocks, plan.schur_shared_w ? 1 : NB, NZ), dim3(64 * plan.schur_waves), plan.schur_lds, stream, dTab, live, maxSlots, plan.schur_shared_w);
         g_baTimer.end(t);
         t = g_baTimer.begin("ba_solve");
-        hipLaunchKernelGGL(k_ba_reduce, dim3((reduceSlots + 31) / 32, NB, NL), dim3(256), 0, stream, dTab, lmBlocks, packedS ? 1 : 0);
-        if (anyMfma64) hipLaunchKernelGGL(k_ba_solve_mfma64, dim3(NB, 1, NL), dim3(64), 0, stream, dTab);
-        if (anyWave) hipLaunchKernelGGL(k_ba_solve_wave, dim3(NB, 1, NL), dim3(64), 0, stream, dTab);
-        if (anyMfma) hipLaunchKernelGGL(k_ba_solve_mfma, dim3(NB, 1, NL), dim3(64 * BA_MFMA_NW), plan.solve_lds, stream, dTab, (double*)nullptr);
+        hipLaunchKernelGGL(k_ba_reduce, dim3((reduceSlots + 31) / 32, candY, NZ), dim3(256), 0, stream, dTab, live, lmBlocks, packedS ? 1 : 0);
+        if (anyMfma64) hipLaunchKernelGGL(k_ba_solve_mfma64, dim3(NB, 1, NZ), dim3(64), 0, stream, dTab, live);
+        if (anyWave) hipLaunchKernelGGL(k_ba_solve_wave, dim3(NB, 1, NZ), dim3(64), 0, stream, dTab, live);
+        if (anyMfma) hipLaunchKernelGGL(k_ba_solve_mfma, dim3(NB, 1, NZ), dim3(64 * BA_MFMA_NW), plan.solve_lds, stream, dTab, live, (double*)nullptr);
         g_baTimer.end(t);
         t = g_baTimer.begin("ba_back");
-        if (useBack2) hipLaunchKernelGGL(k_ba_back2, dim3(plan.back_blocks, 1, NL), dim3(64 * plan.back_waves), plan.back_lds, stream, dTab, maxSlots, maxFac);
-        else hipLaunchKernelGGL(k_ba_back, dim3(plan.back_blocks, plan.back_shared ? 1 : NB, NL), dim3(64 * plan.back_waves), plan.back_lds, stream, dTab, maxSlots, plan.back_shared);
+        if (useBack2) hipLaunchKernelGGL(k_ba_back2, dim3(plan.back_blocks, 1, NZ), dim3(64 * plan.back_waves), plan.back_lds, stream, dTab, live, maxSlots, maxFac);
+        else hipLaunchKernelGGL(k_ba_back, dim3(plan.back_blocks, plan.back_shared ? 1 : NB, NZ), dim3(64 * plan.back_waves), plan.back_lds, stream, dTab, live, maxSlots, plan.back_shared);
         g_baTimer.end(t);
         t = g_baTimer.begin("ba_eval");
-        hipLaunchKernelGGL(k_ba_factors<1>, dim3(facBlocks, NB, NL), dim3(256), 0, stream, dTab, obsBlocks, 1, relTol, absTol);
+        hipLaunchKernelGGL(k_ba_factors<1>, dim3(facBlocks, NB, NZ), dim3(256), 0, stream, dTab, live, obsBlocks, 1, relTol, absTol);
         g_baTimer.end(t);
         VS_HIP(hipGetLastError());
         return VSLAM_OK;
     };
-    double* const b_ctl = (double*)(W.h_back + oBackCtl);
     memcpy(b_ctl, h_ctlAll, (size_t)CTL_DOUBLES * 8 * NL);
     auto lm_loop = [&](int first) -> vslam_status {
         static const int perPollEnv = getenv("VSLAM_BA_STEPS_PER_POLL") ? std::max(1, atoi(getenv("VSLAM_BA_STEPS_PER_POLL"))) : 0;
         int enq = 0, polls = 0;
         for (;;) {
-            const int batch = perPollEnv ? perPollEnv : (enq == 0 ? first : 2);
-            for (int b = 0; b < batch; b++) VS_CHECK(step(enq + b == 0));
+            static const int firstEnv = getenv("VSLAM_BA_FIRST_ROUNDS") ? std::max(1, atoi(getenv("VSLAM_BA_FIRST_ROUNDS"))) : 0;
+            const int batch = perPollEnv ? perPollEnv : (enq == 0 ? (firstEnv ? firstEnv : first) : 2);
+            const BaLive live = live_set();
+            for (int b = 0; b < batch; b++) VS_CHECK(step(enq + b == 0, live));
             enq += batch;
             static const bool mirrorOff = getenv("VSLAM_BA_CTL_MIRROR") && atoi(getenv("VSLAM_BA_CTL_MIRROR")) == 0;
             if (mirrorOff || ++polls > 4) VS_HIP(hipMemcpyAsync(b_ctl, A.dev(h_ctlAll), (size_t)CTL_DOUBLES * 8 * NL, hipMemcpyDeviceToHost, stream));
@@ -3548,6 +3627,7 @@
             R->report[ps].initial_error = c[CTL_INIT_ERR]; R->report[ps].final_error = c[CTL_ERROR]; R->report[ps].lambda = c[CTL_LAMBDA];
             R->n_free_kf = q.H.F;
             R->rounds = (ps == 0 ? 0 : R->rounds) + ci[CI_ROUNDS];
+            g_baLastWork.live_lane_rounds += ci[CI_ROUNDS];
             if (ps == 0) { R->n_residuals = q.H.NF; R->n_landmarks = q.H.Lp; R->sum_k2 = q.H.sumK2; }
             else { R->n_residuals = q.NF2; R->n_landmarks = q.Lp2; R->sum_k2 = q.k2; }
         }
@@ -3661,6 +3741,12 @@
     if (!shape || !plan || shape->n_lanes < 0 || (shape->n_lanes > 0 && !shape->lanes) || shape->lookahead < 1 || shape->lookahead > BA_MAX_NB ||
         shape->solver < 0 || shape->solver > 1) return VSLAM_ERR_INVALID;
     ba_batch_plan(*shape, ba_plan_knobs(), *plan);
+    return VSLAM_OK;
+}
+
+vslam_status vslam_local_ba_last_batch_work(vslam_ba_batch_work* work) {
+    if (!work) return VSLAM_ERR_INVALID;
+    *work = g_baLastWork;
     return VSLAM_OK;
 }
 
diff --git a/gtsam-vslam_amd/vslam_capi.py b/gtsam-vslam_amd/vslam_capi.py
--- a/gtsam-vslam_amd/vslam_capi.py
+++ b/gtsam-vslam_amd/vslam_capi.py
@@ -597,6 +597,16 @@
     P = BaBatchPlan()
     _chk(lib().vslam_local_ba_last_batch_plan(C.byref(P)))
     return _plan_dict(P)
+
+
+class BaBatchWork(C.Structure):
+    _fields_ = [(f, C.c_int64) for f in ("rounds_enqueued", "lane_slots", "live_lane_rounds")]
+
+
+def local_ba_last_batch_work():
+    w = BaBatchWork()
+    _chk(lib().vslam_local_ba_last_batch_work(C.byref(w)))
+    return {f: int(getattr(w, f)) for f, _ in BaBatchWork._fields_}
 
 
 def local_ba_timings():
diff --git a/include/vslam_hip.h b/include/vslam_hip.h
--- a/include/vslam_hip.h
+++ b/include/vslam_hip.h
@@ -365,6 +365,13 @@
 
 vslam_status vslam_local_ba_batch_plan(const vslam_ba_batch_shape* shape, vslam_ba_batch_plan* plan);
 vslam_status vslam_local_ba_last_batch_plan(vslam_ba_batch_plan* plan);
+
+typedef struct vslam_ba_batch_work {
+    int64_t rounds_enqueued;
+    int64_t lane_slots;
+    int64_t live_lane_rounds;
+} vslam_ba_batch_work;
+vslam_status vslam_local_ba_last_batch_work(vslam_ba_batch_work* work);
 
 vslam_status vslam_local_ba(const vslam_ba_problem* problem, vslam_ba_result* result, int32_t device,
                             const vslam_comm* comm);
```

Measured after the change: 29310 (median of 2 runs). About the same (-0.0%).
